# Python-for-HPC/ramba

Hardware: NVIDIA H100
Metric: fused-elementwise GB/s (fp64 sin/cos/mul/add chain) (higher is better)
Workload: dtype f64

## Files before the change

### ramba_b200/csrc/gen_handlers.py

```python
#!/usr/bin/env python

T = ["double", "float", "long long"]
BIN = ["RB200_OP_ADD", "RB200_OP_SUB", "RB200_OP_MUL"]
UN = ["RB200_OP_MOV", "RB200_OP_NEG", "RB200_OP_ABS", "RB200_OP_SQUARE", "RB200_OP_SQRT", "RB200_OP_SIN", "RB200_OP_COS",
      "RB200_OP_SINCOS", "RB200_OP_POWI"]
FLOAT_ONLY = {"RB200_OP_SQRT", "RB200_OP_SIN", "RB200_OP_COS", "RB200_OP_SINCOS", "RB200_OP_POWI"}

SETS = {
    1: dict(AK=["S_ACC", "S_REG", "S_PFV", "S_PFV32"], BK=["S_ACC", "S_REG", "S_SCAL", "S_PFV", "S_PFV32"]),
    2: dict(AK=["S_ACC", "S_REG", "S_VIEW", "S_VIEW32"], BK=["S_ACC", "S_REG", "S_SCAL", "S_VIEW", "S_VIEW32"]),
}


def carr(x):
    if isinstance(x, list):
        return "{" + ", ".join(carr(y) for y in x) + "}"
    return str(x)


tab = ["// GENERATED by gen_handlers.py — do not edit", "#pragma once", "namespace rb200 {"]
for sid, kinds in SETS.items():
    AK, BK = kinds["AK"], kinds["BK"]
    wide32 = {AK[3], BK[4]}
    cases = []
    hid = 0
    hbin = [[[[0] * len(BK) for _ in AK] for _ in T] for _ in BIN]
    hun = [[[0] * len(AK) for _ in T] for _ in UN]
    hred = [[0] * len(AK) for _ in range(2)]
    hcvt = [[[0] * len(AK) for _ in T] for _ in T]
    for ti, t in enumerate(T):
        for group in (lambda op: op not in ("RB200_OP_SIN", "RB200_OP_COS", "RB200_OP_SINCOS"), None,
                      lambda op: op in ("RB200_OP_SIN", "RB200_OP_COS", "RB200_OP_SINCOS")):
            if group is None:
                for oi, op in enumerate(BIN):
                    for ai, ak in enumerate(AK):
                        for bi, bk in enumerate(BK):
                            if (ak in wide32 or bk in wide32) and t != "double":
                                continue
                            hid += 1
                            hbin[oi][ti][ai][bi] = hid
                            cases.append((hid, f"h_bin<{op}, {t}, {ak}, {bk}, V>(cx, I); break;"))
                continue
            for oi, op in enumerate(UN):
                if not group(op):
                    continue
                if op in FLOAT_ONLY and t == "long long":
                    continue
                for ai, ak in enumerate(AK):
                    if ak in wide32 and t != "double":
                        continue
                    hid += 1
                    hun[oi][ti][ai] = hid
                    cases.append((hid, f"h_un<{op}, {t}, {ak}, V>(cx, I); break;"))
    for ti, t in enumerate(["double", "long long"]):
        for ai, ak in enumerate(AK):
            if ak in wide32 and t != "double":
                continue
            hid += 1
            hred[ti][ai] = hid
            cases.append((hid, f"h_red<{t}, {ak}, V, AX, NS>(cx, I, racc); break;"))
    for si, ts in enumerate(T):
        for di, td in enumerate(T):
            if si == di:
                continue
            for ai, ak in enumerate(AK[:3]):
                hid += 1
                hcvt[si][di][ai] = hid
                cases.append((hid, f"h_cvt<{ts}, {td}, {ak}, V>(cx, I); break;"))
    groups = {}
    for n, stmt in cases:
        groups.setdefault(n >> 4, []).append((n & 15, stmt))
    lines = ["// GENERATED by gen_handlers.py — do not edit", "switch (h >> 4) {"]
    for gi in sorted(groups):
        lines.append(f"  case {gi}:")
        lines.append("    switch (h & 15) {")
        for lo, stmt in groups[gi]:
            lines.append(f"      case {lo}: {stmt}")
        lines.append("      default: break;")
        lines.append("    }")
        lines.append("    break;")
    lines.append("  default: break;")
    lines.append("}")
    open(f"rb200_handlers_set{sid}.inc", "w").write("\n".join(lines) + "\n")
    tab += [f"// ---- set {sid}: a kinds {AK}, b kinds {BK}",
            f"constexpr int kNumHandlers{sid} = {hid};",
            f"static const short kHandlerBin{sid}[{len(BIN)}][{len(T)}][{len(AK)}][{len(BK)}] = {carr(hbin)};",
            f"static const short kHandlerUn{sid}[{len(UN)}][{len(T)}][{len(AK)}] = {carr(hun)};",
            f"static const short kHandlerRed{sid}[2][{len(AK)}] = {carr(hred)};",
            f"static const short kHandlerCvt{sid}[{len(T)}][{len(T)}][{len(AK)}] = {carr(hcvt)};"]
    print("set", sid, hid, "handlers")
tab += ["}  // namespace rb200", ""]
open("rb200_handler_tables.h", "w").write("\n".join(tab))
```

### ramba_b200/csrc/rb200_api.cu

```cuda
#include <cuda_runtime.h>
#include <math.h>
#include <stdio.h>
#include <stdlib.h>
#include <string.h>
#include <atomic>
#include <string>

#include "rb200_launch.h"
#include "rb200_handlers.h"
#include "rb200_group.h"
#include "rb200_index.h"
#include "rb200_rng.h"
#include "rb200_stream.h"
#include "rb200_tile.h"

namespace rb200 {
__global__ void fill_u64_kernel(u64* p, long long n, u64 bits) {
  for (long long i = (long long)blockIdx.x * blockDim.x + threadIdx.x; i < n; i += (long long)gridDim.x * blockDim.x) p[i] = bits;
}

template <class T> __global__ void reduce_partials_kernel(T* out, const T* part, long long n, long long k, long long stride_k, int op) {
  for (long long j = (long long)blockIdx.x * blockDim.x + threadIdx.x; j < n; j += (long long)gridDim.x * blockDim.x) {
    T v = part[j];
    for (long long q = 1; q < k; ++q) v = red_combine<T>(op, v, part[q * stride_k + j]);
    out[j] = v;
  }
}

}

using namespace rb200;

static thread_local std::string g_last_error;
static std::atomic<long long> g_launches{0};

static int fail(const std::string& msg) {
  g_last_error = msg;
  return 1;
}
static int fail_cuda(const char* what, cudaError_t e) {
  g_last_error = std::string(what) + ": " + cudaGetErrorString(e);
  return 2;
}

static int dtype_size(int dt) {
  switch (dt) {
    case RB200_F64:
    case RB200_I64: return 8;
    case RB200_F32:
    case RB200_I32:
    case RB200_U32: return 4;
    case RB200_I16:
    case RB200_U16: return 2;
    case RB200_BOOL:
    case RB200_U8:
    case RB200_I8: return 1;
    default: return 0;
  }
}

static std::atomic<int> g_sm_count{0};
static int sm_count() {
  const int cached = g_sm_count.load();
  if (cached > 0) return cached;
  int dev = 0;
  if (cudaGetDevice(&dev) != cudaSuccess) return -1;
  int n = 0;
  if (cudaDeviceGetAttribute(&n, cudaDevAttrMultiProcessorCount, dev) != cudaSuccess) return -1;
  g_sm_count.store(n);
  return n;
}

constexpr int kRedScratchPartials = 4096;

static int static_kind(const KParams& P, int set, int kind, int* idx, int ctype) {
  switch (kind) {
    case RB200_K_ACC: return S_ACC;
    case RB200_K_REG: return S_REG;
    case RB200_K_SCAL: return S_SCAL;
    case RB200_K_VIEW: {
      const KView& v = P.views[*idx];
      const int own = ctype == RB200_T_F64 ? RB200_F64 : ctype == RB200_T_F32 ? RB200_F32 : RB200_I64;
      if (set == 2) {
        if (v.dtype == own) return S_VIEW;
        if (ctype == RB200_T_F64 && v.dtype == RB200_F32) return S_VIEW32;
        return -1;
      }
      if (v.pf_slot < 0) return -1;
      if (v.dtype == own) {
        *idx = v.pf_slot;
        return S_PFV;
      }
      if (ctype == RB200_T_F64 && v.dtype == RB200_F32) {
        *idx = v.pf_slot;
        return S_PFV32;
      }
      return -1;
    }
    default: return -1;
  }
}

static unsigned long long host_red_identity_bits(int op, int ctype) {
  if (ctype == RB200_T_F64) {
    double d = (op == RB200_RED_ADD) ? 0.0 : (op == RB200_RED_MUL) ? 1.0 : (op == RB200_RED_MIN) ? INFINITY : -INFINITY;
    unsigned long long b;
    memcpy(&b, &d, 8);
    return b;
  }
  long long i = (op == RB200_RED_ADD) ? 0ll : (op == RB200_RED_MUL) ? 1ll : (op == RB200_RED_MIN) ? 0x7fffffffffffffffll : (long long)0x8000000000000000ull;
  return (unsigned long long)i;
}

static void assign_handlers(KParams& P, const rb200_fused_op* op, int set) {
  for (int i = 0; i < P.n_insns; ++i) {
    rb200_insn I = P.insns[i];
    int h = H_GENERIC;
    int ai = I.a_idx, bi = I.b_idx;
    const int ak = static_kind(P, set, I.a_kind, &ai, I.op == RB200_OP_CVT ? (int)(I.imm & 0xff) : (int)I.ctype);
    if (I.op == RB200_OP_ADD || I.op == RB200_OP_SUB || I.op == RB200_OP_MUL) {
      const int bk = static_kind(P, set, I.b_kind, &bi, I.ctype);
      h = handler_bin(set, I.op, I.ctype, ak, bk);
    } else if (I.op == RB200_OP_RED) {
      h = handler_red(set, I.ctype, ak);
    } else if (I.op == RB200_OP_CVT) {
      if ((I.imm >> 8) == 0) h = handler_cvt(set, (int)(I.imm & 0xff), I.ctype, ak);
    } else if (I.op == RB200_OP_POWI) {
      if (I.b_kind == RB200_K_SCAL && (long long)op->scalars[I.b_idx] == 2) h = handler_un(set, I.op, I.ctype, ak);
    } else if ((I.c_kind == RB200_K_NONE || I.op == RB200_OP_SINCOS) && I.b_kind == RB200_K_NONE) {
      h = handler_un(set, I.op, I.ctype, ak);
    }
    if (h != H_GENERIC) {
      I.a_idx = (uint8_t)ai;
      if (I.op != RB200_OP_RED) I.b_idx = (uint8_t)bi;
      P.insns[i] = I;
    }
    P.handler[i] = (unsigned short)h;
  }
}

struct KillSwitches {
  bool no_tile, no_stream, no_mapred, no_terms, no_tma, no_row_mode, no_rng;
};
static const KillSwitches& kill_switches() {
  static const KillSwitches k = {getenv("RB200_NO_TILE_KERNEL") != nullptr,   getenv("RB200_NO_STREAM_KERNEL") != nullptr,
                                 getenv("RB200_NO_MAPRED_KERNEL") != nullptr, getenv("RB200_NO_TERMS_KERNEL") != nullptr,
                                 getenv("RB200_NO_TMA") != nullptr,           getenv("RB200_NO_ROW_MODE") != nullptr,
                                 getenv("RB200_NO_RNG") != nullptr};
  return k;
}

static int validate(const rb200_fused_op* op, bool* empty) {
  if (!op) return fail("null fused op");
  if (op->abi_version != RB200_ABI_VERSION) return fail("ABI version mismatch between caller and libramba_b200");
  if (op->ndim < 1 || op->ndim > RB200_MAX_DIMS) return fail("ndim out of range");
  if (op->n_views < 0 || op->n_views > RB200_MAX_VIEWS) return fail("too many views");
  if (op->n_scalars < 0 || op->n_scalars > RB200_MAX_SCALARS) return fail("too many scalars");
  if (op->n_insns < 0 || op->n_insns > RB200_MAX_INSNS) return fail("too many instructions");
  if (op->n_regs < 0 || op->n_regs > RB200_MAX_REGS) return fail("too many spill registers");
  if (op->n_reds < 0 || op->n_reds > RB200_MAX_REDS) return fail("too many reductions");
  long long total = 1;
  for (int d = 0; d < op->ndim; ++d) {
    if (op->itershape[d] < 0) return fail("negative itershape");
    if (op->ndim > 1 && op->itershape[d] >= (1ll << 31)) return fail("N-d iteration dims must be < 2^31");
    total *= op->itershape[d];
  }
  *empty = total == 0 || op->n_insns == 0;
  if (*empty) return 0;

  for (int i = 0; i < op->n_insns; ++i) {
    const rb200_insn& I = op->insns[i];
    if (I.op >= RB200_NUM_OPS) return fail("bad opcode");
    if (I.ctype > RB200_T_I64) return fail("bad compute class");
    const uint8_t kinds[3] = {I.a_kind, I.b_kind, I.c_kind};
    const uint8_t idxs[3] = {I.a_idx, I.b_idx, I.c_idx};
    for (int q = 0; q < 3; ++q) {
      if (I.op == RB200_OP_RED && q == 1) continue;
      if (I.op == RB200_OP_SINCOS && q == 2) {
        if (kinds[q] == RB200_K_VIEW && idxs[q] >= op->n_views) return fail("view index out of range");
        continue;
      }
      switch (kinds[q]) {
        case RB200_K_NONE:
        case RB200_K_ACC: break;
        case RB200_K_REG: if (idxs[q] >= op->n_regs) return fail("register index out of range"); break;
        case RB200_K_VIEW: if (idxs[q] >= op->n_views) return fail("view index out of range"); break;
        case RB200_K_SCAL: if (idxs[q] >= op->n_scalars) return fail("scalar index out of range"); break;
        case RB200_K_IOTA: if (idxs[q] >= op->ndim) return fail("iota dim out of range"); break;
        default: return fail("bad operand kind");
      }
    }
    if (I.st_reg != RB200_NOSTORE && I.st_reg >= op->n_regs) return fail("st_reg out of range");
    if (I.st_view != RB200_NOSTORE && I.st_view >= op->n_views) return fail("st_view out of range");
    if (I.mask_reg != RB200_NOSTORE && I.mask_reg >= op->n_regs) return fail("mask_reg out of range");
    if (I.op == RB200_OP_SINCOS && I.st2 >= op->n_regs) return fail("sincos st2 out of range");
    if (I.op == RB200_OP_RED && I.b_idx >= op->n_reds) return fail("reduction slot out of range");
    if (I.op == RB200_OP_PHILOX) {
      if (I.imm > RB200_PHILOX_INTEGER) return fail("philox: bad output form");
      const int cls = I.imm == RB200_PHILOX_UNIFORM32 ? RB200_T_F32 : I.imm == RB200_PHILOX_INTEGER ? RB200_T_I64 : RB200_T_F64;
      if (I.ctype != cls) return fail("philox: compute class does not match the output form");
      if (I.a_kind != RB200_K_IOTA && I.a_kind != RB200_K_ACC && I.a_kind != RB200_K_REG) return fail("philox: the index must be an index, the accumulator or a register");
      if (I.b_kind != RB200_K_SCAL) return fail("philox: the key must be a scalar");
      if (I.imm == RB200_PHILOX_INTEGER) {
        if (I.c_kind != RB200_K_SCAL) return fail("philox: the integer form needs a scalar bound");
        if ((long long)op->scalars[I.c_idx] <= 0) return fail("philox: the bound must be positive");
      }
    }
  }
  for (int i = 0; i < op->n_views; ++i) {
    if (dtype_size(op->views[i].dtype) == 0) return fail("bad view dtype");
    if (!op->views[i].base) return fail("null view base pointer");
  }
  if (op->n_axis_red_dims != 0) {
    if (op->n_axis_red_dims >= op->ndim) return fail("axis reduction needs at least one kept dim");
    if (op->n_reds < 1) return fail("axis reduction without reduction slots");
    if (!op->red_scratch) return fail("axis reduction needs a partial buffer");
  } else if (op->n_reds > 0) {
    if (!op->red_scratch) return fail("global reduction needs red_scratch");
    for (int s = 0; s < op->n_reds; ++s) {
      if (!op->reds[s].out) return fail("null reduction output");
      if (dtype_size(op->reds[s].out_dtype) == 0) return fail("bad reduction output dtype");
      if (op->reds[s].ctype != RB200_T_F64 && op->reds[s].ctype != RB200_T_I64) return fail("reduction class must be F64 or I64");
    }
  }
  return 0;
}

enum PlanForm { FORM_NONE, FORM_TILE, FORM_STREAM, FORM_AXIS_AS_1D, FORM_AXIS_REDUCE, FORM_ELEMENTWISE, FORM_RNG };

struct Plan {
  PlanForm form;
  TilePlan tile;
  StreamPlan stream;
  RngPlan rng;
  KParams k;
  long long blocks;
  size_t smem;
  int n_split, n_written;
  long long kept;
  u64* partials;
  u64 identity;
};

static bool plan_axis_as_1d(const rb200_fused_op* op, int sms, const bool* view_read, size_t reg_bytes, Plan& pl) {
  const KParams& P = pl.k;
  const long long TILE1 = (long long)kThreads * kV1;
  const long long red_len = P.red_len, kept = P.total;
  bool ok = (op->ndim == 2 && P.red_ndim == 1 && op->n_reds == 1 && kept % TILE1 == 0 && kept / TILE1 <= (long long)sms * 2 && red_len >= 2);
  for (int i = 0; i < op->n_insns && ok; ++i) {
    const rb200_insn& I = op->insns[i];
    if (I.a_kind == RB200_K_IOTA || I.b_kind == RB200_K_IOTA || I.c_kind == RB200_K_IOTA) ok = false;
    if (I.st_view != RB200_NOSTORE) ok = false;
    if (I.op == RB200_OP_SINCOS && I.c_kind == RB200_K_VIEW) ok = false;
  }
  for (int i = 0; i < op->n_views && ok; ++i) {
    const rb200_view& v = op->views[i];
    if (!view_read[i]) continue;
    if (v.stride[1] != 1 || !(v.stride[0] == kept || v.stride[0] == 0)) ok = false;
  }
  if (!ok) return false;
  KParams Q = P;
  const int V1 = kV1;
  Q.ndim = 1;
  Q.total = red_len * kept;
  Q.n_tiles = Q.total / TILE1;
  Q.shape[0] = Q.total;
  Q.gstart[0] = 0;
  Q.wide = 1;
  const int n_chunks = (int)(kept / TILE1);
  long long cap1 = (long long)sms * 2;
  int n_split_eff = (int)(cap1 / n_chunks);
  if (n_split_eff > P.n_split) n_split_eff = P.n_split;
  if ((long long)n_split_eff > red_len) n_split_eff = (int)red_len;
  if (n_split_eff < 1) n_split_eff = 1;
  Q.n_split_chunks = n_chunks;
  Q.n_split = n_split_eff;
  Q.red_len = kept;
  Q.n_pf = 0;
  for (int i = 0; i < op->n_views; ++i) {
    KView& k = Q.views[i];
    const rb200_view& v = op->views[i];
    k.stride[0] = 1;
    k.pf_slot = -1;
    if (!view_read[i]) continue;
    const int dt = v.dtype;
    const bool wide_ok = (dt == RB200_F64 || dt == RB200_F32 || dt == RB200_I64 || dt == RB200_I32);
    if (v.stride[0] == 0) {
      k.pf_slot = -2;
    } else if (wide_ok && Q.n_pf < kMaxPf && reg_bytes + (size_t)(Q.n_pf + 1) * 2 * V1 * kThreads * 8 <= 108 * 1024) {
      k.pf_slot = Q.n_pf;
      Q.pf_view[Q.n_pf] = i;
      Q.n_pf++;
    }
  }
  for (int i = 0; i < op->n_views && Q.n_hoist < kMaxPf; ++i) {
    if (Q.views[i].pf_slot != -2 || Q.n_regs >= RB200_MAX_REGS) continue;
    int cls = -1;
    bool same = true;
    for (int q = 0; q < Q.n_insns; ++q) {
      const rb200_insn& I = Q.insns[q];
      const int use_cls = (I.op == RB200_OP_CVT) ? (int)(I.imm & 0xff) : (int)I.ctype;
      const bool uses = (I.a_kind == RB200_K_VIEW && I.a_idx == i) || (I.b_kind == RB200_K_VIEW && I.b_idx == i && I.op != RB200_OP_RED) ||
                        (I.c_kind == RB200_K_VIEW && I.c_idx == i && I.op != RB200_OP_SINCOS);
      if (!uses) continue;
      if (I.op == RB200_OP_POWI && I.b_kind == RB200_K_VIEW && I.b_idx == i) same = false;
      if (cls < 0) cls = use_cls;
      else if (cls != use_cls) same = false;
    }
    if (cls < 0 || !same) continue;
    const int r = Q.n_regs++;
    Q.hoist_view[Q.n_hoist] = i;
    Q.hoist_reg[Q.n_hoist] = r;
    Q.hoist_cls[Q.n_hoist] = cls;
    Q.n_hoist++;
    for (int q = 0; q < Q.n_insns; ++q) {
      rb200_insn& I = Q.insns[q];
      if (I.a_kind == RB200_K_VIEW && I.a_idx == i) { I.a_kind = RB200_K_REG; I.a_idx = (uint8_t)r; }
      if (I.b_kind == RB200_K_VIEW && I.b_idx == i && I.op != RB200_OP_RED) { I.b_kind = RB200_K_REG; I.b_idx = (uint8_t)r; }
      if (I.c_kind == RB200_K_VIEW && I.c_idx == i && I.op != RB200_OP_SINCOS) { I.c_kind = RB200_K_REG; I.c_idx = (uint8_t)r; }
    }
  }
  const size_t reg_bytes1 = (size_t)(Q.n_regs + 1) * V1 * kThreads * 8;
  Q.bulk = Q.n_pf > 0 ? 1 : 0;
  for (int j = 0; j < Q.n_pf; ++j)
    if ((((uintptr_t)op->views[Q.pf_view[j]].base) & 15u) != 0) Q.bulk = 0;
  Q.n_stages = 2;
  const size_t pf_bytes1 = (size_t)Q.n_pf * Q.n_stages * V1 * kThreads * 8;
  if (reg_bytes1 + pf_bytes1 > 200 * 1024) return false;
  assign_handlers(Q, op, 1);
  pl.k = Q;
  pl.form = FORM_AXIS_AS_1D;
  pl.blocks = (long long)n_split_eff * n_chunks;
  pl.smem = reg_bytes1 + pf_bytes1;
  pl.n_written = n_split_eff;
  return true;
}

static void make_plan(const rb200_fused_op* op, int sms, Plan& pl) {
  const KillSwitches& ks = kill_switches();
  pl.form = FORM_NONE;
  pl.n_split = pl.n_written = 0;
  if (!ks.no_rng && plan_rng(op, sms, pl.rng)) {
    pl.form = FORM_RNG;
    return;
  }
  if (!ks.no_tile && plan_stencil_tile(op, sms, !ks.no_terms, !ks.no_tma, pl.tile)) {
    pl.form = FORM_TILE;
    return;
  }
  if (op->ndim == 1 && op->n_axis_red_dims == 0 && !ks.no_stream &&
      plan_stream(op, sms, kRedScratchPartials, 0, !ks.no_terms, !ks.no_mapred, pl.stream)) {
    pl.form = FORM_STREAM;
    return;
  }

  const int V = (op->ndim == 1 && op->n_axis_red_dims == 0) ? kV1 : kV;
  const long long TILE = (long long)kThreads * V;
  KParams& P = pl.k;
  memset(&P, 0, sizeof(P));
  P.ndim = op->ndim;
  P.n_insns = op->n_insns;
  P.n_views = op->n_views;
  P.n_regs = op->n_regs;
  P.n_reds = op->n_reds;
  long long total = 1;
  for (int d = 0; d < op->ndim; ++d) {
    P.shape[d] = op->itershape[d];
    P.gstart[d] = op->global_start[d];
    total *= op->itershape[d];
  }
  bool view_read[RB200_MAX_VIEWS] = {false}, view_masked[RB200_MAX_VIEWS] = {false};
  for (int i = 0; i < op->n_insns; ++i) {
    const rb200_insn& I = op->insns[i];
    const uint8_t kinds[3] = {I.a_kind, I.b_kind, I.c_kind};
    const uint8_t idxs[3] = {I.a_idx, I.b_idx, I.c_idx};
    for (int q = 0; q < 3; ++q)
      if (kinds[q] == RB200_K_VIEW && !(I.op == RB200_OP_RED && q == 1) && !(I.op == RB200_OP_SINCOS && q == 2)) view_read[idxs[q]] = true;
    if (I.st_view != RB200_NOSTORE && I.mask_reg != RB200_NOSTORE) view_masked[I.st_view] = true;
    P.insns[i] = I;
  }
  for (int i = 0; i < op->n_scalars; ++i) P.scalars[i] = op->scalars[i];
  for (int i = 0; i < op->n_views; ++i) {
    const rb200_view& v = op->views[i];
    KView& k = P.views[i];
    k.base = (char*)v.base;
    k.dtype = v.dtype;
    k.pf_slot = -1;
    for (int d = 0; d < op->ndim; ++d) k.stride[d] = v.stride[d];
  }
  const size_t reg_bytes = (size_t)(op->n_regs + 1) * V * kThreads * 8;

  if (op->n_axis_red_dims != 0) {
    const int nred = op->n_axis_red_dims;
    P.red_ndim = nred;
    long long red_len = 1, kept = 1;
    for (int d = 0; d < nred; ++d) red_len *= P.shape[d];
    for (int d = nred; d < op->ndim; ++d) kept *= P.shape[d];
    int n_split = op->axis_nsplit;
    if (n_split < 1) n_split = 1;
    if ((long long)n_split > red_len) n_split = (int)red_len;
    P.red_len = red_len;
    P.n_split = n_split;
    P.red_split = (red_len + n_split - 1) / n_split;
    P.total = kept;
    P.n_tiles = ((kept + TILE - 1) / TILE) * n_split;
    P.red_partials = (u64*)op->red_scratch;
    for (int s = 0; s < op->n_reds; ++s) {
      P.reds[s].op = op->reds[s].op;
      P.reds[s].ctype = op->reds[s].ctype;
    }
    pl.n_split = n_split;
    pl.kept = kept;
    pl.partials = (u64*)op->red_scratch;
    pl.identity = host_red_identity_bits(op->reds[0].op, op->reds[0].ctype);
    if (!ks.no_stream && plan_stream(op, sms, kRedScratchPartials, n_split, !ks.no_terms, !ks.no_mapred, pl.stream)) {
      pl.form = FORM_STREAM;
      pl.n_written = pl.stream.eff;
      return;
    }
    if (plan_axis_as_1d(op, sms, view_read, reg_bytes, pl)) return;
    long long blocks = P.n_tiles;
    long long cap = (long long)sms * 4;
    if (blocks > cap) blocks = cap;
    pl.form = FORM_AXIS_REDUCE;
    pl.blocks = blocks;
    pl.smem = reg_bytes;
    pl.n_written = n_split;
    return;
  }

  P.total = total;
  P.n_tiles = (total + TILE - 1) / TILE;
  P.row_chunks = 0;
  if (op->ndim > 1) {
    const long long inner = op->itershape[op->ndim - 1];
    const long long chunks = (inner + TILE - 1) / TILE;
    if (!ks.no_row_mode && inner * 5 >= chunks * TILE * 4 && chunks < (1ll << 30)) {
      P.row_chunks = (int)chunks;
      P.n_tiles = (total / inner) * chunks;
    }
  }
  P.wide = (total >= (1ll << 31)) ? 1 : 0;
  size_t pf_bytes = 0;
  if (op->ndim == 1) {
    for (int i = 0; i < op->n_views && P.n_pf < kMaxPf; ++i) {
      const int dt = op->views[i].dtype;
      const bool wide_ok = (dt == RB200_F64 || dt == RB200_F32 || dt == RB200_I64 || dt == RB200_I32);
      if (view_read[i] && !view_masked[i] && wide_ok && reg_bytes + (size_t)(P.n_pf + 1) * 2 * V * kThreads * 8 <= 108 * 1024) {
        P.views[i].pf_slot = P.n_pf;
        P.pf_view[P.n_pf] = i;
        P.n_pf++;
      }
    }
    P.n_stages = 2;
    pf_bytes = (size_t)P.n_pf * P.n_stages * V * kThreads * 8;
    P.bulk = P.n_pf > 0 ? 1 : 0;
    for (int j = 0; j < P.n_pf; ++j) {
      const rb200_view& v = op->views[P.pf_view[j]];
      if (v.stride[0] != 1 || (((uintptr_t)v.base) & 15u) != 0) P.bulk = 0;
    }
  }
  size_t ocls_bytes = 0;
  if (op->ndim > 1) {
    for (int i = 0; i < op->n_views; ++i) {
      int c = -1;
      for (int q = 0; q < P.n_ocls && c < 0; ++q) {
        bool same = true;
        for (int d = 0; d < op->ndim; ++d)
          if (op->views[P.ocls_view[q]].stride[d] != op->views[i].stride[d]) same = false;
        if (same) c = q;
      }
      if (c < 0 && P.n_ocls < kMaxOcls) {
        c = P.n_ocls;
        P.ocls_view[P.n_ocls++] = i;
      }
      P.views[i].pf_slot = c;
    }
    ocls_bytes = (size_t)P.n_ocls * V * kThreads * 8;
  }
  const size_t smem = reg_bytes + pf_bytes + ocls_bytes;
  assign_handlers(P, op, op->ndim == 1 ? 1 : 2);
  if (op->n_reds > 0) {
    P.red_counter = (unsigned int*)op->red_scratch;
    P.red_partials = (u64*)((char*)op->red_scratch + 256);
    for (int s = 0; s < op->n_reds; ++s) {
      P.reds[s].op = op->reds[s].op;
      P.reds[s].ctype = op->reds[s].ctype;
      P.reds[s].out = op->reds[s].out;
      P.reds[s].out_dtype = op->reds[s].out_dtype;
    }
  }
  int per_sm = (V == 4 && op->ndim == 1) ? 3 : 2;
  if (smem > 0) {
    int by_smem = (int)((220 * 1024) / (smem + 1024));
    if (by_smem < 1) by_smem = 1;
    if (per_sm > by_smem) per_sm = by_smem;
  }
  long long blocks = P.n_tiles;
  long long cap = (long long)sms * per_sm;
  if (op->n_reds > 0 && cap > kRedScratchPartials) cap = kRedScratchPartials;
  if (blocks > cap) blocks = cap;
  pl.form = FORM_ELEMENTWISE;
  pl.blocks = blocks;
  pl.smem = smem;
}

static std::string launch_failure(const Plan& pl) {
  const KParams& P = pl.k;
  char buf[256];
  switch (pl.form) {
    case FORM_TILE: {
      const TilePlan& T = pl.tile;
      snprintf(buf, sizeof(buf), "stencil_tile_kernel launch (blocks=%lld smem=%zu group=%d tma=%d)", T.blocks, T.smem, T.P.has_group, T.P.use_tma);
    } break;
    case FORM_STREAM: {
      const StreamPlan& T = pl.stream;
      snprintf(buf, sizeof(buf), "stream kernel%s launch (blocks=%lld smem=%zu staged=%d depth=%d terms=%d)", T.P.mode == 1 ? " (columns)" : "", T.blocks,
               T.smem, T.P.n_staged, T.P.depth, T.P.n_terms);
    } break;
    case FORM_RNG: snprintf(buf, sizeof(buf), "rng_fill_kernel launch (blocks=%lld)", pl.rng.blocks); break;
    case FORM_AXIS_AS_1D: return "vm_elementwise_kernel (axis-as-1-D) launch";
    case FORM_AXIS_REDUCE: return "vm_axis_reduce_kernel launch";
    default:
      snprintf(buf, sizeof(buf), "vm_elementwise_kernel launch (ndim=%d blocks=%lld smem=%zu n_regs=%d n_pf=%d n_insns=%d)", P.ndim, pl.blocks, pl.smem,
               P.n_regs, P.n_pf, P.n_insns);
  }
  return buf;
}

static int launch(Plan& pl, cudaStream_t stream) {
  const KParams& P = pl.k;
  const unsigned blocks = (unsigned)pl.blocks;
  cudaError_t e = cudaSuccess;
  switch (pl.form) {
    case FORM_NONE: return 0;
    case FORM_TILE: e = launch_stencil_tile(pl.tile, stream); break;
    case FORM_STREAM: e = launch_stream(pl.stream, stream); break;
    case FORM_RNG: e = launch_rng(pl.rng, stream); break;
    case FORM_AXIS_AS_1D: e = launch_vm_elementwise_ax1d(P, blocks, pl.smem, stream); break;
    case FORM_AXIS_REDUCE: e = launch_vm_axis_reduce(P, blocks, pl.smem, stream); break;
    case FORM_ELEMENTWISE:
      switch (P.ndim) {
        case 1: e = launch_vm_elementwise_nd1(P, blocks, pl.smem, stream); break;
        case 2: e = launch_vm_elementwise_nd2(P, blocks, pl.smem, stream); break;
        case 3: e = launch_vm_elementwise_nd3(P, blocks, pl.smem, stream); break;
        default: e = launch_vm_elementwise_nd5(P, blocks, pl.smem, stream); break;
      }
      break;
  }
  if (e != cudaSuccess) return fail_cuda(launch_failure(pl).c_str(), e);
  g_launches.fetch_add(1);
  if (pl.n_written < pl.n_split) {
    const long long n_fill = (long long)(pl.n_split - pl.n_written) * pl.kept;
    fill_u64_kernel<<<(unsigned)((n_fill + 255) / 256 > 1184 ? 1184 : (n_fill + 255) / 256), 256, 0, stream>>>(pl.partials + (long long)pl.n_written * pl.kept,
                                                                                                               n_fill, pl.identity);
    e = cudaGetLastError();
    if (e != cudaSuccess) return fail_cuda("fill_u64_kernel launch", e);
    g_launches.fetch_add(1);
  }
  return 0;
}

static std::string describe(const rb200_fused_op* op, const Plan& pl) {
  if (pl.form == FORM_TILE) return describe_stencil_tile(pl.tile);
  if (pl.form == FORM_STREAM) return describe_stream(pl.stream);
  if (pl.form == FORM_RNG) return describe_rng(pl.rng);
  if (pl.form == FORM_NONE) return "kernel=none";
  const char* form = pl.form == FORM_ELEMENTWISE ? "elementwise" : pl.form == FORM_AXIS_AS_1D ? "axis_as_1d" : "axis_reduce";
  const char* tiling = pl.form != FORM_ELEMENTWISE || op->ndim == 1 ? "" : pl.k.row_chunks > 0 ? " tiling=row" : " tiling=flat";
  char buf[200];
  snprintf(buf, sizeof(buf), "kernel=general_interpreter form=%s ndim=%d insns=%d views=%d%s ctas=%lld smem=%zu", form, op->ndim, op->n_insns, op->n_views,
           tiling, pl.blocks, pl.smem);
  return buf;
}

static int check_index_view(const rb200_index_view* v, const char* who) {
  const std::string w(who);
  if (!v) return fail(w + ": null view");
  if (v->elem_bytes != 1 && v->elem_bytes != 2 && v->elem_bytes != 4 && v->elem_bytes != 8) return fail(w + ": elem_bytes must be 1, 2, 4 or 8");
  if (v->ndim < 1 || v->ndim > RB200_MAX_DIMS) return fail(w + ": ndim out of range");
  long long size = 1, lo = 0, hi = 0;
  for (int d = 0; d < v->ndim; ++d) {
    if (v->shape[d] < 0) return fail(w + ": negative shape");
    size *= v->shape[d];
    const long long reach = (v->shape[d] > 0 ? v->shape[d] - 1 : 0) * v->stride[d];
    if (reach < 0) lo += reach;
    else hi += reach;
  }
  if (size == 0) return 0;
  if (!v->base) return fail(w + ": null view base pointer");
  if (v->alloc_lo && v->alloc_hi) {
    const char* b = (const char*)v->base;
    if (b + lo * v->elem_bytes < (const char*)v->alloc_lo || b + (hi + 1) * v->elem_bytes > (const char*)v->alloc_hi)
      return fail(w + ": view outside its allocation");
  }
  return 0;
}

static int check_route_table(const rb200_route_table* t, RouteParams* R) {
  if (!t) return fail("route: null table");
  if (t->ndim < 1 || t->ndim > RB200_MAX_DIMS) return fail("route: ndim out of range");
  if (t->n_ranks < 1 || t->n_ranks > RB200_MAX_ROUTE_RANKS) return fail("route: too many ranks (or none)");
  if (!t->cuts || !t->cell_owner || !t->cell_offset || !t->cell_stride) return fail("route: null table array");
  R->ndim = t->ndim;
  R->n_ranks = t->n_ranks;
  R->size = 1;
  long long n_cells = 1;
  int n_cuts = 0;
  for (int d = 0; d < t->ndim; ++d) {
    if (t->shape[d] < 0) return fail("route: negative shape");
    if (t->n_cells[d] < 1) return fail("route: not a grid (no cells along a dim)");
    R->shape[d] = t->shape[d];
    R->size *= t->shape[d];
    n_cells *= t->n_cells[d];
    R->n_cells[d] = t->n_cells[d];
    R->cut_start[d] = n_cuts;
    const int first = t->cut_start[d], m = t->n_cells[d] + 1;
    if (first < 0 || n_cuts + m > RB200_MAX_ROUTE_CUTS) return fail("route: too many cut points");
    if (n_cells > RB200_MAX_ROUTE_CELLS) return fail("route: too many cells");
    for (int j = 0; j < m; ++j) R->cuts[n_cuts + j] = t->cuts[first + j];
    if (R->cuts[n_cuts] != 0 || R->cuts[n_cuts + m - 1] != t->shape[d]) return fail("route: not a grid (cuts must run from 0 to the extent)");
    for (int j = 1; j < m; ++j)
      if (R->cuts[n_cuts + j] <= R->cuts[n_cuts + j - 1] && t->shape[d] > 0) return fail("route: not a grid (cuts must ascend)");
    n_cuts += m;
  }
  for (long long c = 0; c < n_cells; ++c) {
    if (t->cell_owner[c] < 0 || t->cell_owner[c] >= t->n_ranks) return fail("route: cell owner out of range");
    R->owner[c] = t->cell_owner[c];
    R->offset[c] = t->cell_offset[c];
    for (int d = 0; d < t->ndim; ++d) R->stride[c * t->ndim + d] = t->cell_stride[c * t->ndim + d];
  }
  return 0;
}

static int check_group_args(const rb200_index_view* src, int axis, int n_groups, GroupPlan* P) {
  if (const int rc = check_index_view(src, "group_reduce")) return rc;
  if (axis < 0 || axis >= src->ndim) return fail("group_reduce: axis out of range");
  if (n_groups < 1) return fail("group_reduce: n_groups must be >= 1");
  make_group_plan(*src, axis, n_groups, P);
  if (P->ctas >= (1ll << 31)) return fail("group_reduce: too many outputs for one launch");
  return 0;
}

static thread_local std::string g_group_plan_text;

extern "C" {

const char* rb200_last_error(void) { return g_last_error.c_str(); }
int rb200_abi_version(void) { return RB200_ABI_VERSION; }
int64_t rb200_launch_count(void) { return (int64_t)g_launches.load(); }
void rb200_reset_launch_count(void) { g_launches.store(0); }
int rb200_device_sm_count(void) { return sm_count(); }
int64_t rb200_red_scratch_bytes(void) { return (int64_t)(256 + 8 * RB200_MAX_REDS * kRedScratchPartials); }

int rb200_run_deferred_ops(const rb200_fused_op* op, void* stream_v) {
  bool empty = false;
  if (const int rc = validate(op, &empty)) return rc;
  if (empty) return 0;
  const int sms = sm_count();
  if (sms <= 0) return fail("no usable CUDA device (libramba_b200 has no CPU path)");
  Plan pl;
  make_plan(op, sms, pl);
  return launch(pl, (cudaStream_t)stream_v);
}

int rb200_describe_plan(const rb200_fused_op* op, char* out, int64_t cap) {
  if (!out || cap < 2) return fail("describe_plan: null argument");
  bool empty = false;
  if (const int rc = validate(op, &empty)) return rc;
  Plan pl;
  pl.form = FORM_NONE;
  if (!empty) make_plan(op, 132, pl);
  snprintf(out, (size_t)cap, "%s", describe(op, pl).c_str());
  return 0;
}

int64_t rb200_cumulative_scratch_bytes(int64_t n_outer, int64_t len, int64_t n_inner) {
  if (n_outer < 0 || len < 0 || n_inner < 1) return 256;
  return (int64_t)scan_scratch_bytes(n_outer, len, n_inner);
}

int rb200_cumulative(const void* src, void* dst, int32_t dtype, int64_t n_outer, int64_t len, int64_t n_inner, int32_t redop, const void* carry_in,
                     void* totals_out, void* scratch, void* stream_v) {
  if (n_outer < 0 || len < 0 || n_inner < 1) return fail("cumulative: bad extents");
  if (redop < RB200_RED_ADD || redop > RB200_RED_MAX) return fail("cumulative: bad operation");
  if (dtype != RB200_F64 && dtype != RB200_F32 && dtype != RB200_I64 && dtype != RB200_I32) return fail("cumulative: dtype must be float64/float32/int64/int32");
  if (n_outer == 0 || len == 0) return 0;
  if (!src || !dst || !scratch) return fail("null pointer");
  const int sms = sm_count();
  if (sms <= 0) return fail("no usable CUDA device (libramba_b200 has no CPU path)");
  bool supported = true;
  const cudaError_t e = launch_scan(src, dst, dtype, n_outer, len, n_inner, redop, carry_in, totals_out, scratch, sms, (cudaStream_t)stream_v, &supported);
  if (!supported) return fail("cumulative: unsupported dtype");
  if (e != cudaSuccess) return fail_cuda("scan kernel launch", e);
  g_launches.fetch_add(1);
  return 0;
}

int rb200_gather(const rb200_index_view* view, const int64_t* lin, int64_t n, void* out, uint64_t* bad, void* stream_v) {
  if (const int rc = check_index_view(view, "gather")) return rc;
  if (n < 0) return fail("gather: negative n");
  if (n == 0) return 0;
  if (!lin || !out || !bad) return fail("gather: null pointer");
  const int sms = sm_count();
  if (sms <= 0) return fail("no usable CUDA device (libramba_b200 has no CPU path)");
  const cudaError_t e = launch_gather(collapse_index_view(*view), (const long long*)lin, n, out, (unsigned long long*)bad, sms, (cudaStream_t)stream_v);
  if (e != cudaSuccess) return fail_cuda("gather kernel launch", e);
  g_launches.fetch_add(1);
  return 0;
}

int rb200_scatter(const rb200_index_view* view, const int64_t* lin, int64_t n, const void* values, uint64_t* bad, void* stream_v) {
  if (const int rc = check_index_view(view, "scatter")) return rc;
  if (n < 0) return fail("scatter: negative n");
  if (n == 0) return 0;
  if (!lin || !values || !bad) return fail("scatter: null pointer");
  const int sms = sm_count();
  if (sms <= 0) return fail("no usable CUDA device (libramba_b200 has no CPU path)");
  const cudaError_t e =
      launch_scatter(collapse_index_view(*view), (const long long*)lin, n, values, (unsigned long long*)bad, sms, (cudaStream_t)stream_v);
  if (e != cudaSuccess) return fail_cuda("scatter kernel launch", e);
  g_launches.fetch_add(1);
  return 0;
}

int64_t rb200_route_scratch_bytes(int64_t n, int32_t n_ranks) {
  if (n < 0 || n_ranks < 1) return 256;
  return (int64_t)route_scratch_bytes(n, n_ranks);
}

int rb200_route(const rb200_route_table* table, const int64_t* lin, int64_t n, int64_t* offsets, int64_t* slots, int64_t* counts, uint64_t* bad,
                void* scratch, void* stream_v) {
  RouteParams R;
  if (const int rc = check_route_table(table, &R)) return rc;
  if (n < 0) return fail("route: negative n");
  if (!counts || !scratch) return fail("route: null pointer");
  if (n > 0 && (!lin || !offsets || !slots || !bad)) return fail("route: null pointer");
  const int sms = sm_count();
  if (sms <= 0) return fail("no usable CUDA device (libramba_b200 has no CPU path)");
  const cudaError_t e = launch_route(R, (const long long*)lin, n, (long long*)offsets, (long long*)slots, (long long*)counts,
                                     (unsigned long long*)bad, scratch, sms, (cudaStream_t)stream_v);
  if (e != cudaSuccess) return fail_cuda("route kernel launch", e);
  g_launches.fetch_add(1);
  return 0;
}

int64_t rb200_group_reduce_scratch_bytes(const rb200_index_view* src, int32_t axis, int32_t n_groups) {
  GroupPlan P;
  if (check_group_args(src, axis, n_groups, &P)) return -1;
  return (int64_t)P.scratch_bytes;
}

const char* rb200_describe_group_plan(const rb200_index_view* src, int32_t axis, int32_t n_groups) {
  GroupPlan P;
  if (check_group_args(src, axis, n_groups, &P)) return nullptr;
  char buf[240];
  snprintf(buf, sizeof(buf), "kernel=group form=%s chunk=%lld chunks=%d cta_chunks=%d ctas_per_row=%d kept=%lld groups=%d ctas=%lld scratch=%lld",
           group_form_name(P.form), P.C, P.S, P.ncl, P.K, P.nkept, P.G, P.ctas, P.scratch_bytes);
  g_group_plan_text = buf;
  return g_group_plan_text.c_str();
}

int rb200_group_reduce(const rb200_index_view* src, int32_t src_dtype, int32_t axis, const rb200_group_table* groups, int32_t op, const void* center,
                       void* out, void* scratch, void* stream_v) {
  if (op < 0 || op >= RB200_GROUP_NUM_OPS) return fail("group_reduce: bad op");
  if (src_dtype != RB200_F64 && src_dtype != RB200_F32 && src_dtype != RB200_I64 && src_dtype != RB200_I32)
    return fail("group_reduce: source dtype must be float64, float32, int64 or int32");
  if (src && dtype_size(src_dtype) != src->elem_bytes) return fail("group_reduce: elem_bytes does not match the source dtype");
  if (!groups) return fail("group_reduce: null group table");
  GroupPlan P;
  if (const int rc = check_group_args(src, axis, groups->n_groups, &P)) return rc;
  if (groups->len != src->shape[axis]) return fail("group_reduce: table len differs from the extent of the grouped axis");
  if (!groups->offsets || (groups->len > 0 && !groups->members)) return fail("group_reduce: null table array");
  if (op == RB200_GROUP_SQDEV && !center) return fail("group_reduce: SQDEV needs center");
  if (!out) return fail("group_reduce: null out");
  if (P.scratch_bytes && !scratch) return fail("group_reduce: null scratch (this plan splits the axis)");
  if (P.nkept == 0) return 0;
  const int sms = sm_count();
  if (sms <= 0) return fail("no usable CUDA device (libramba_b200 has no CPU path)");
  const cudaError_t e = launch_group(P, src_dtype, op, (const long long*)groups->offsets, (const long long*)groups->members, (const double*)center, out,
                                     scratch, (cudaStream_t)stream_v);
  if (e != cudaSuccess) return fail_cuda("group kernel launch", e);
  g_launches.fetch_add(1);
  return 0;
}

int rb200_reduce_partials(void* out, const void* partials, int64_t n, int64_t k, int64_t stride_k, int32_t dtype,
                          int32_t redop, void* stream_v) {
  if (!out || !partials) return fail("null pointer");
  if (n <= 0 || k <= 0) return 0;
  const int sms = sm_count();
  if (sms <= 0) return fail("no usable CUDA device (libramba_b200 has no CPU path)");
  cudaStream_t stream = (cudaStream_t)stream_v;
  long long blocks = (n + 255) / 256;
  if (blocks > sms * 8) blocks = sms * 8;
  if (dtype == RB200_F64)
    reduce_partials_kernel<double><<<(unsigned)blocks, 256, 0, stream>>>((double*)out, (const double*)partials, n, k, stride_k, redop);
  else if (dtype == RB200_I64)
    reduce_partials_kernel<long long><<<(unsigned)blocks, 256, 0, stream>>>((long long*)out, (const long long*)partials, n, k, stride_k, redop);
  else
    return fail("reduce_partials: dtype must be F64 or I64 (accumulator classes)");
  cudaError_t e = cudaGetLastError();
  if (e != cudaSuccess) return fail_cuda("reduce_partials_kernel launch", e);
  g_launches.fetch_add(1);
  return 0;
}

}
```

### ramba_b200/csrc/rb200_elementwise.cuh

```cuda
#pragma once
#include "rb200_interp.cuh"
#include "rb200_launch.h"

namespace rb200 {

template <int V, int ND, bool AX1D = false>
#ifndef RB200_MIN_BLOCKS
#define RB200_MIN_BLOCKS 2
#endif
__global__ void __launch_bounds__(kThreads, (ND == 1 && V <= 4) ? 3 : RB200_MIN_BLOCKS) vm_elementwise_kernel(const __grid_constant__ KParams P) {
  extern __shared__ __align__(128) unsigned char smem[];
  __shared__ __align__(8) u64 mbar_store[4];
  constexpr int TILE = kThreads * V;
  constexpr unsigned SLOT = (unsigned)(TILE * 8);
  Ctx<V, ND> cx(P);
  const unsigned smem_s = (unsigned)__cvta_generic_to_shared(smem);
  cx.tid = threadIdx.x;
  const int n_pf = (ND == 1) ? P.n_pf : 0;
  const unsigned pf_base = smem_s;
  const unsigned pf_stage_bytes = (unsigned)n_pf * SLOT;
  const bool bulk = (ND == 1) && n_pf > 0 && P.bulk;
  constexpr unsigned S = 2u;
  cx.regfile_s = smem_s + (n_pf > 0 ? S : 0u) * pf_stage_bytes + threadIdx.x * 8u;
  cx.ocls_s = cx.regfile_s + (unsigned)((P.n_regs + 1) * V * kThreads * 8);
  cx.pf_s = pf_base;
  const unsigned mbar0 = (unsigned)__cvta_generic_to_shared(&mbar_store[0]);
  if (bulk) {
    if (threadIdx.x == 0) {
      for (unsigned s = 0; s < S; ++s) mbar_init(mbar0 + s * 8u, 1);
      asm volatile("fence.mbarrier_init.release.cluster;" ::: "memory");
    }
    __syncthreads();
  }

  constexpr int NS = 1;
  __shared__ u64 racc_extra[RB200_MAX_REDS - 1][kThreads];
  u64 racc[NS][AX1D ? V : 1];
#pragma unroll
  for (int k = 0; k < (AX1D ? V : 1); ++k) racc[0][k] = red_identity_bits(0 < P.n_reds ? P.reds[0].op : 0, 0 < P.n_reds ? P.reds[0].ctype : 0);
  cx.racc_s = (unsigned)__cvta_generic_to_shared(&racc_extra[0][threadIdx.x]);
  for (int s = 1; s < P.n_reds; ++s) racc_extra[s - 1][threadIdx.x] = red_identity_bits(P.reds[s].op, P.reds[s].ctype);
  if constexpr (AX1D) {
    cx.pe0 = (long long)(blockIdx.x % (unsigned)P.n_split_chunks) * TILE + threadIdx.x;
    cx.e0 = cx.pe0;
    cx.valid = (1u << V) - 1u;
#pragma unroll 1
    for (int h = 0; h < P.n_hoist; ++h) {
      const KView& vw = P.views[P.hoist_view[h]];
      long long off[V];
      cx.offsets(vw, off);
      u64 bits[V];
      if (P.hoist_cls[h] == RB200_T_F64) {
        double t[V];
        load_view<double, V>(vw.base, vw.dtype, off, cx.valid, t);
#pragma unroll
        for (int k = 0; k < V; ++k) bits[k] = CT<double>::bits(t[k]);
      } else if (P.hoist_cls[h] == RB200_T_F32) {
        float t[V];
        load_view<float, V>(vw.base, vw.dtype, off, cx.valid, t);
#pragma unroll
        for (int k = 0; k < V; ++k) bits[k] = CT<float>::bits(t[k]);
      } else {
        long long t[V];
        load_view<long long, V>(vw.base, vw.dtype, off, cx.valid, t);
#pragma unroll
        for (int k = 0; k < V; ++k) bits[k] = CT<long long>::bits(t[k]);
      }
      sts_vec64<V>(cx.reg_base(P.hoist_reg[h]), bits);
    }
  } else {
    cx.pe0 = 0;
  }

  auto issue_bulk = [&](long long t, unsigned st) {
    const unsigned mb = mbar0 + st * 8u;
    unsigned bytes = 0;
#pragma unroll 1
    for (int j = 0; j < n_pf; ++j) {
      const int dt = P.views[P.pf_view[j]].dtype;
      bytes += (unsigned)TILE * ((dt == RB200_F64 || dt == RB200_I64) ? 8u : 4u);
    }
    mbar_expect_tx(mb, bytes);
#pragma unroll 1
    for (int j = 0; j < n_pf; ++j) {
      const KView& vw = P.views[P.pf_view[j]];
      const unsigned es = (vw.dtype == RB200_F64 || vw.dtype == RB200_I64) ? 8u : 4u;
      bulk_g2s(pf_base + st * pf_stage_bytes + (unsigned)j * SLOT, vw.base + t * (long long)TILE * es, (unsigned)TILE * es, mb);
    }
  };
  auto issue_ldgsts = [&](long long t, unsigned st) {
    const long long e0 = t * TILE + threadIdx.x;
    const long long left = P.total - e0;
#pragma unroll 1
    for (int j = 0; j < n_pf; ++j) {
      const KView& vw = P.views[P.pf_view[j]];
      const int es = (vw.dtype == RB200_F64 || vw.dtype == RB200_I64) ? 8 : 4;
      const long long sb = vw.stride[0] * es;
      const long long step = sb * kThreads;
      const char* src = vw.base + e0 * sb;
      unsigned dst = pf_base + st * pf_stage_bytes + (unsigned)j * SLOT + threadIdx.x * (unsigned)es;
#pragma unroll
      for (int k = 0; k < V; ++k) {
        const bool ok = (long long)k * kThreads < left;
        if (es == 8) cp_async8(dst, ok ? src : vw.base, ok);
        else cp_async4(dst, ok ? src : vw.base, ok);
        src += step;
        dst += (unsigned)(kThreads * es);
      }
    }
  };
  auto tile_is_bulk = [&](long long t) { return bulk && (t + 1) * TILE <= P.total; };

  constexpr unsigned lgS = 1u;
  if (n_pf > 0 && (long long)blockIdx.x < P.n_tiles) {
    if (bulk) {
      if (threadIdx.x == 0) {
        long long t = blockIdx.x;
        for (unsigned s = 0; s < S && t < P.n_tiles; ++s, t += gridDim.x)
          if (tile_is_bulk(t)) issue_bulk(t, s);
      }
    } else {
      issue_ldgsts(blockIdx.x, 0);
      cp_async_commit();
    }
  }
#pragma unroll 1
  for (unsigned it = 0;; ++it) {
    unsigned grid = gridDim.x;
    asm volatile("" : "+r"(grid));
    const long long tile = (long long)blockIdx.x + (long long)it * grid;
    if (tile >= P.n_tiles) break;
    const unsigned stage = bulk ? (it & (S - 1u)) : (it & 1u);
    if (n_pf > 0) {
      if (bulk) {
        __syncthreads();
        if (it > 0 && threadIdx.x == 0) {
          const long long nxt = tile + (long long)(S - 1u) * grid;
          if (nxt < P.n_tiles && tile_is_bulk(nxt)) issue_bulk(nxt, (it - 1u) & (S - 1u));
        }
        if (tile_is_bulk(tile)) {
          mbar_wait(mbar0 + stage * 8u, (it >> lgS) & 1u);
        } else {
          issue_ldgsts(tile, stage);
          cp_async_commit();
          cp_async_wait<0>();
        }
      } else {
        const long long nxt = tile + grid;
        if (nxt < P.n_tiles) issue_ldgsts(nxt, stage ^ 1u);
        cp_async_commit();
        cp_async_wait<1>();
      }
      cx.pf_s = pf_base + stage * pf_stage_bytes;
    }
    const long long e0 = tile * TILE + threadIdx.x;
    unsigned valid = 0;
    if constexpr (ND == 1) {
      cx.e0 = e0;
      if ((tile + 1) * TILE <= P.total) {
        valid = (1u << V) - 1u;
      } else {
#pragma unroll
        for (int k = 0; k < V; ++k)
          if (e0 + (long long)k * kThreads < P.total) valid |= (1u << k);
      }
    } else if (P.row_chunks > 0) {
      long long row, ch;
      if (((tile | (long long)P.row_chunks) >> 31) == 0) row = (long long)((unsigned)tile / (unsigned)P.row_chunks);
      else row = tile / P.row_chunks;
      ch = tile - row * P.row_chunks;
      long long oidx[ND];
#pragma unroll
      for (int d = ND - 1; d >= 0; --d) {
        if (d >= P.ndim - 1) {
          oidx[d] = 0;
        } else if (d == 0) {
          oidx[d] = row;
        } else {
          const long long sd = P.shape[d];
          long long q;
          if (((row | sd) >> 31) == 0) q = (long long)((unsigned)row / (unsigned)sd);
          else q = row / sd;
          oidx[d] = row - q * sd;
          row = q;
        }
      }
      const long long inner = P.shape[P.ndim - 1];
      const long long j0 = ch * TILE + threadIdx.x;
#pragma unroll
      for (int k = 0; k < V; ++k) {
        const long long j = j0 + (long long)k * kThreads;
        const bool ok = j < inner;
        if (ok) valid |= (1u << k);
#pragma unroll
        for (int d = 0; d < ND; ++d) cx.idx[k][d] = (d == P.ndim - 1) ? (ok ? j : 0) : (ok ? oidx[d] : 0);
      }
    } else {
#pragma unroll
      for (int k = 0; k < V; ++k) {
        const long long e = e0 + (long long)k * kThreads;
        if (e < P.total) {
          valid |= (1u << k);
          decode_index<ND>(P, e, 0, cx.idx[k]);
        } else {
#pragma unroll
          for (int d = 0; d < ND; ++d) cx.idx[k][d] = 0;
        }
      }
    }
    cx.valid = valid;
    cx.fill_offset_classes();
    run_program<V, AX1D, NS>(cx, racc);
  }
  if (n_pf > 0 && !bulk) cp_async_wait<0>();

  if constexpr (AX1D) {
    const long long split = blockIdx.x / (unsigned)P.n_split_chunks;
    const long long col0 = cx.pe0;
#pragma unroll
    for (int k = 0; k < V; ++k) P.red_partials[split * P.red_len + col0 + (long long)k * kThreads] = racc[0][k];
    return;
  }
  if (P.n_reds > 0) {
    __shared__ u64 wpart[RB200_MAX_REDS][kThreads / 32];
    __shared__ bool is_last;
    const int lane = threadIdx.x & 31, warp = threadIdx.x >> 5;
    for (int s = 0; s < P.n_reds; ++s) {
      const int op = P.reds[s].op, ct = P.reds[s].ctype;
      u64 v = (s == 0) ? racc[0][0] : racc_extra[s > 0 ? s - 1 : 0][threadIdx.x];
#pragma unroll
      for (int o = 16; o > 0; o >>= 1) v = red_combine_bits(op, ct, v, __shfl_down_sync(0xffffffffu, v, o));
      if (lane == 0) wpart[s][warp] = v;
    }
    __syncthreads();
    if (threadIdx.x == 0) {
      for (int s = 0; s < P.n_reds; ++s) {
        const int op = P.reds[s].op, ct = P.reds[s].ctype;
        u64 v = wpart[s][0];
        for (int q = 1; q < kThreads / 32; ++q) v = red_combine_bits(op, ct, v, wpart[s][q]);
        P.red_partials[(long long)s * gridDim.x + blockIdx.x] = v;
      }
      __threadfence();
      unsigned prev = atomicAdd(P.red_counter, 1u);
      is_last = (prev == gridDim.x - 1);
    }
    __syncthreads();
    if (is_last) {
      __threadfence();
      for (int s = 0; s < P.n_reds; ++s) {
        const int op = P.reds[s].op, ct = P.reds[s].ctype;
        u64 v = red_identity_bits(op, ct);
        for (unsigned b = threadIdx.x; b < gridDim.x; b += kThreads) v = red_combine_bits(op, ct, v, __ldcg(&P.red_partials[(long long)s * gridDim.x + b]));
#pragma unroll
        for (int o = 16; o > 0; o >>= 1) v = red_combine_bits(op, ct, v, __shfl_down_sync(0xffffffffu, v, o));
        __syncthreads();
        if (lane == 0) wpart[s][warp] = v;
        __syncthreads();
        if (threadIdx.x == 0) {
          v = wpart[s][0];
          for (int q = 1; q < kThreads / 32; ++q) v = red_combine_bits(op, ct, v, wpart[s][q]);
          void* out = P.reds[s].out;
          const double vd = (ct == RB200_T_F64) ? CT<double>::get(v) : (double)(long long)v;
          const long long vi = (ct == RB200_T_F64) ? (long long)CT<double>::get(v) : (long long)v;
          switch (P.reds[s].out_dtype) {
            case RB200_F64: { double* o = (double*)out; *o = red_combine<double>(op, *o, vd); } break;
            case RB200_F32: { float* o = (float*)out; *o = (float)red_combine<double>(op, (double)*o, vd); } break;
            case RB200_I64: { long long* o = (long long*)out; *o = red_combine<long long>(op, *o, vi); } break;
            case RB200_I32: { int* o = (int*)out; *o = (int)red_combine<long long>(op, (long long)*o, vi); } break;
            case RB200_BOOL: { unsigned char* o = (unsigned char*)out; *o = red_combine<long long>(op, (long long)*o, vi) != 0 ? 1 : 0; } break;
            case RB200_U8: { unsigned char* o = (unsigned char*)out; *o = (unsigned char)red_combine<long long>(op, (long long)*o, vi); } break;
            case RB200_I8: { signed char* o = (signed char*)out; *o = (signed char)red_combine<long long>(op, (long long)*o, vi); } break;
            case RB200_I16: { short* o = (short*)out; *o = (short)red_combine<long long>(op, (long long)*o, vi); } break;
            case RB200_U16: { unsigned short* o = (unsigned short*)out; *o = (unsigned short)red_combine<long long>(op, (long long)*o, vi); } break;
            case RB200_U32: { unsigned int* o = (unsigned int*)out; *o = (unsigned int)red_combine<long long>(op, (long long)*o, vi); } break;
            default: break;
          }
        }
      }
      if (threadIdx.x == 0) *P.red_counter = 0u;
    }
  }
}

template <int V, int ND, bool AX1D = false> cudaError_t launch_vm_elementwise_nd(const KParams& P, unsigned blocks, size_t smem, cudaStream_t stream) {
  if (smem + 2048 > 48 * 1024) {
    cudaError_t e = cudaFuncSetAttribute(vm_elementwise_kernel<V, ND, AX1D>, cudaFuncAttributeMaxDynamicSharedMemorySize, (int)smem);
    if (e != cudaSuccess) return e;
  }
  vm_elementwise_kernel<V, ND, AX1D><<<blocks, kThreads, smem, stream>>>(P);
  return cudaGetLastError();
}

}
```

### ramba_b200/csrc/rb200_handler_tables.h

```cpp
#pragma once
namespace rb200 {
constexpr int kNumHandlers1 = 232;
static const short kHandlerBin1[3][3][4][5] = {{{{25, 26, 27, 28, 29}, {30, 31, 32, 33, 34}, {35, 36, 37, 38, 39}, {40, 41, 42, 43, 44}}, {{115, 116, 117, 118, 0}, {119, 120, 121, 122, 0}, {123, 124, 125, 126, 0}, {0, 0, 0, 0, 0}}, {{172, 173, 174, 175, 0}, {176, 177, 178, 179, 0}, {180, 181, 182, 183, 0}, {0, 0, 0, 0, 0}}}, {{{45, 46, 47, 48, 49}, {50, 51, 52, 53, 54}, {55, 56, 57, 58, 59}, {60, 61, 62, 63, 64}}, {{127, 128, 129, 130, 0}, {131, 132, 133, 134, 0}, {135, 136, 137, 138, 0}, {0, 0, 0, 0, 0}}, {{184, 185, 186, 187, 0}, {188, 189, 190, 191, 0}, {192, 193, 194, 195, 0}, {0, 0, 0, 0, 0}}}, {{{65, 66, 67, 68, 69}, {70, 71, 72, 73, 74}, {75, 76, 77, 78, 79}, {80, 81, 82, 83, 84}}, {{139, 140, 141, 142, 0}, {143, 144, 145, 146, 0}, {147, 148, 149, 150, 0}, {0, 0, 0, 0, 0}}, {{196, 197, 198, 199, 0}, {200, 201, 202, 203, 0}, {204, 205, 206, 207, 0}, {0, 0, 0, 0, 0}}}};
static const short kHandlerUn1[9][3][4] = {{{1, 2, 3, 4}, {97, 98, 99, 0}, {160, 161, 162, 0}}, {{5, 6, 7, 8}, {100, 101, 102, 0}, {163, 164, 165, 0}}, {{9, 10, 11, 12}, {103, 104, 105, 0}, {166, 167, 168, 0}}, {{13, 14, 15, 16}, {106, 107, 108, 0}, {169, 170, 171, 0}}, {{17, 18, 19, 20}, {109, 110, 111, 0}, {0, 0, 0, 0}}, {{85, 86, 87, 88}, {151, 152, 153, 0}, {0, 0, 0, 0}}, {{89, 90, 91, 92}, {154, 155, 156, 0}, {0, 0, 0, 0}}, {{93, 94, 95, 96}, {157, 158, 159, 0}, {0, 0, 0, 0}}, {{21, 22, 23, 24}, {112, 113, 114, 0}, {0, 0, 0, 0}}};
static const short kHandlerRed1[2][4] = {{208, 209, 210, 211}, {212, 213, 214, 0}};
static const short kHandlerCvt1[3][3][4] = {{{0, 0, 0, 0}, {215, 216, 217, 0}, {218, 219, 220, 0}}, {{221, 222, 223, 0}, {0, 0, 0, 0}, {224, 225, 226, 0}}, {{227, 228, 229, 0}, {230, 231, 232, 0}, {0, 0, 0, 0}}};
constexpr int kNumHandlers2 = 232;
static const short kHandlerBin2[3][3][4][5] = {{{{25, 26, 27, 28, 29}, {30, 31, 32, 33, 34}, {35, 36, 37, 38, 39}, {40, 41, 42, 43, 44}}, {{115, 116, 117, 118, 0}, {119, 120, 121, 122, 0}, {123, 124, 125, 126, 0}, {0, 0, 0, 0, 0}}, {{172, 173, 174, 175, 0}, {176, 177, 178, 179, 0}, {180, 181, 182, 183, 0}, {0, 0, 0, 0, 0}}}, {{{45, 46, 47, 48, 49}, {50, 51, 52, 53, 54}, {55, 56, 57, 58, 59}, {60, 61, 62, 63, 64}}, {{127, 128, 129, 130, 0}, {131, 132, 133, 134, 0}, {135, 136, 137, 138, 0}, {0, 0, 0, 0, 0}}, {{184, 185, 186, 187, 0}, {188, 189, 190, 191, 0}, {192, 193, 194, 195, 0}, {0, 0, 0, 0, 0}}}, {{{65, 66, 67, 68, 69}, {70, 71, 72, 73, 74}, {75, 76, 77, 78, 79}, {80, 81, 82, 83, 84}}, {{139, 140, 141, 142, 0}, {143, 144, 145, 146, 0}, {147, 148, 149, 150, 0}, {0, 0, 0, 0, 0}}, {{196, 197, 198, 199, 0}, {200, 201, 202, 203, 0}, {204, 205, 206, 207, 0}, {0, 0, 0, 0, 0}}}};
static const short kHandlerUn2[9][3][4] = {{{1, 2, 3, 4}, {97, 98, 99, 0}, {160, 161, 162, 0}}, {{5, 6, 7, 8}, {100, 101, 102, 0}, {163, 164, 165, 0}}, {{9, 10, 11, 12}, {103, 104, 105, 0}, {166, 167, 168, 0}}, {{13, 14, 15, 16}, {106, 107, 108, 0}, {169, 170, 171, 0}}, {{17, 18, 19, 20}, {109, 110, 111, 0}, {0, 0, 0, 0}}, {{85, 86, 87, 88}, {151, 152, 153, 0}, {0, 0, 0, 0}}, {{89, 90, 91, 92}, {154, 155, 156, 0}, {0, 0, 0, 0}}, {{93, 94, 95, 96}, {157, 158, 159, 0}, {0, 0, 0, 0}}, {{21, 22, 23, 24}, {112, 113, 114, 0}, {0, 0, 0, 0}}};
static const short kHandlerRed2[2][4] = {{208, 209, 210, 211}, {212, 213, 214, 0}};
static const short kHandlerCvt2[3][3][4] = {{{0, 0, 0, 0}, {215, 216, 217, 0}, {218, 219, 220, 0}}, {{221, 222, 223, 0}, {0, 0, 0, 0}, {224, 225, 226, 0}}, {{227, 228, 229, 0}, {230, 231, 232, 0}, {0, 0, 0, 0}}};
}
```

### ramba_b200/csrc/rb200_interp.cuh

```cuda
#pragma once
#include <cuda_runtime.h>
#include <math.h>
#include <type_traits>

#include "rb200_vm.cuh"
#include "rb200_handlers.h"
#include "rb200_philox.h"

namespace rb200 {

struct UInsn {
  uint2 lo, hi;
  __device__ __forceinline__ UInsn(const rb200_insn* p) {
    lo = *reinterpret_cast<const uint2*>(p);
    hi = *(reinterpret_cast<const uint2*>(p) + 1);
  }
  __device__ __forceinline__ unsigned op() const { return lo.x & 0xffu; }
  __device__ __forceinline__ unsigned ctype() const { return (lo.x >> 8) & 0xffu; }
  __device__ __forceinline__ unsigned a_kind() const { return (lo.x >> 16) & 0xffu; }
  __device__ __forceinline__ unsigned a_idx() const { return lo.x >> 24; }
  __device__ __forceinline__ unsigned b_kind() const { return lo.y & 0xffu; }
  __device__ __forceinline__ unsigned b_idx() const { return (lo.y >> 8) & 0xffu; }
  __device__ __forceinline__ unsigned c_kind() const { return (lo.y >> 16) & 0xffu; }
  __device__ __forceinline__ unsigned c_idx() const { return lo.y >> 24; }
  __device__ __forceinline__ unsigned st_reg() const { return hi.x & 0xffu; }
  __device__ __forceinline__ unsigned st_view() const { return (hi.x >> 8) & 0xffu; }
  __device__ __forceinline__ unsigned st2() const { return (hi.x >> 16) & 0xffu; }
  __device__ __forceinline__ unsigned mask_reg() const { return hi.x >> 24; }
  __device__ __forceinline__ unsigned imm() const { return hi.y; }
};

template <class T, int V, int K = 0> __device__ __forceinline__ void lds_vec64(unsigned base, T (&out)[V]) {
  if constexpr (K < V) {
    out[K] = CT<T>::get(lds64o<K * kThreads * 8>(base));
    lds_vec64<T, V, K + 1>(base, out);
  }
}
template <class T, int V, int K = 0> __device__ __forceinline__ void lds_vec32(unsigned base, T (&out)[V]) {
  if constexpr (K < V) {
    out[K] = CT<T>::get((u64)lds32o<K * kThreads * 4>(base));
    lds_vec32<T, V, K + 1>(base, out);
  }
}
template <int V, int K = 0> __device__ __forceinline__ void lds_vec32_as_f64(unsigned base, double (&out)[V]) {
  if constexpr (K < V) {
    out[K] = (double)__uint_as_float(lds32o<K * kThreads * 4>(base));
    lds_vec32_as_f64<V, K + 1>(base, out);
  }
}
template <int V, int K = 0> __device__ __forceinline__ void sts_vec64(unsigned base, const u64 (&v)[V]) {
  if constexpr (K < V) {
    sts64o<K * kThreads * 8>(base, v[K]);
    sts_vec64<V, K + 1>(base, v);
  }
}

template <class R>
__device__ __noinline__ void store_line(char* base, int dtype, long long off0, long long step, unsigned mask, u64 b0, u64 b1, u64 b2, u64 b3) {
  constexpr int V = 4;
  long long off[V] = {off0, off0 + step, off0 + 2 * step, off0 + 3 * step};
  R r[V] = {CT<R>::get(b0), CT<R>::get(b1), CT<R>::get(b2), CT<R>::get(b3)};
  constexpr int own = std::is_same<R, double>::value ? RB200_F64 : std::is_same<R, float>::value ? RB200_F32 : RB200_I64;
  if (dtype == own) {
    store_direct<R, R, V>(base, off, mask, r);
  } else if (dtype == RB200_BOOL) {
    long long b[V];
#pragma unroll
    for (int k = 0; k < V; ++k) b[k] = (r[k] != R(0)) ? 1 : 0;
    store_view<long long, V>(base, RB200_U8, off, mask, b);
  } else {
    store_view<R, V>(base, dtype, off, mask, r);
  }
}

template <class R> __device__ __forceinline__ void store_one(char* base, int dtype, long long off, R x) {
  switch (dtype) {
    case RB200_F64: reinterpret_cast<double*>(base)[off] = (double)x; break;
    case RB200_F32: reinterpret_cast<float*>(base)[off] = (float)x; break;
    case RB200_I64: reinterpret_cast<long long*>(base)[off] = (long long)x; break;
    case RB200_I32: reinterpret_cast<int*>(base)[off] = (int)x; break;
    default: store_narrow_one<R>(base, dtype, off, x);
  }
}

template <class R, int V>
__device__ __noinline__ void store_slow_1d(char* base, int dtype, long long stride, long long e0, unsigned valid, unsigned mask_addr,
                                           unsigned vals_addr) {
  const long long step = stride * kThreads;
  long long off = e0 * stride;
#pragma unroll 1
  for (int k = 0; k < V; ++k, off += step) {
    if (!((valid >> k) & 1u)) continue;
    if (mask_addr != 0xffffffffu && lds64(mask_addr + (unsigned)(k * kThreads * 8)) == 0ull) continue;
    store_one<R>(base, dtype, off, CT<R>::get(lds64(vals_addr + (unsigned)(k * kThreads * 8))));
  }
}

template <class R>
__device__ __noinline__ void store_slow_nd(char* base, int dtype, unsigned mask, long long o0, long long o1, long long o2, long long o3,
                                           unsigned vals_addr) {
  if (mask & 1u) store_one<R>(base, dtype, o0, CT<R>::get(lds64(vals_addr)));
  if (mask & 2u) store_one<R>(base, dtype, o1, CT<R>::get(lds64(vals_addr + (unsigned)(kThreads * 8))));
  if (mask & 4u) store_one<R>(base, dtype, o2, CT<R>::get(lds64(vals_addr + (unsigned)(2 * kThreads * 8))));
  if (mask & 8u) store_one<R>(base, dtype, o3, CT<R>::get(lds64(vals_addr + (unsigned)(3 * kThreads * 8))));
}

template <int V, int ND> struct Ctx {
  static constexpr int kND = ND;
  const KParams& P;
  unsigned regfile_s;
  unsigned racc_s;
  unsigned pf_s;
  unsigned ocls_s;
  unsigned tid;
  long long e0;
  long long pe0;
  long long idx[V][ND];
  unsigned valid;
  u64 acc[V];

  __device__ __forceinline__ Ctx(const KParams& p) : P(p) {}

  __device__ __forceinline__ void offsets(const KView& vw, long long (&off)[V]) const {
    if constexpr (ND == 1) {
      const long long s = vw.stride[0];
      const long long step = s * kThreads;
      long long o = (vw.pf_slot == -2 ? pe0 : e0) * s;
#pragma unroll
      for (int k = 0; k < V; ++k) {
        off[k] = o;
        o += step;
      }
    } else {
      const int c = vw.pf_slot;
      if (c >= 0) {
        lds_vec64<long long, V>(ocls_s + (unsigned)(c * V * kThreads * 8), off);
        return;
      }
      compute_offsets(vw, off);
    }
  }
  __device__ __forceinline__ void compute_offsets(const KView& vw, long long (&off)[V]) const {
    if constexpr (ND > 1) {
#pragma unroll
      for (int k = 0; k < V; ++k) {
        long long o = 0;
#pragma unroll
        for (int d = 0; d < ND; ++d) o += idx[k][d] * vw.stride[d];
        off[k] = o;
      }
    }
  }
  __device__ __forceinline__ void fill_offset_classes() {
    if constexpr (ND > 1) {
#pragma unroll 1
      for (int c = 0; c < P.n_ocls; ++c) {
        long long off[V];
        compute_offsets(P.views[P.ocls_view[c]], off);
        u64 b[V];
#pragma unroll
        for (int k = 0; k < V; ++k) b[k] = (u64)off[k];
        sts_vec64<V>(ocls_s + (unsigned)(c * V * kThreads * 8), b);
      }
    }
  }

  __device__ __forceinline__ unsigned reg_addr(int r, int k) const { return regfile_s + (unsigned)((r * V + k) * kThreads * 8); }
  __device__ __forceinline__ unsigned reg_base(int r) const { return regfile_s + (unsigned)(r * V * kThreads * 8); }

  template <class T> __device__ __forceinline__ void fetch(int kind, int i, T (&out)[V]) {
    switch (kind) {
      case RB200_K_ACC:
#pragma unroll
        for (int k = 0; k < V; ++k) out[k] = CT<T>::get(acc[k]);
        break;
      case RB200_K_REG:
#pragma unroll
        for (int k = 0; k < V; ++k) out[k] = CT<T>::get(lds64(reg_addr(i, k)));
        break;
      case RB200_K_VIEW: {
        const KView& vw = P.views[i];
        const int slot = vw.pf_slot;
        const int dt = vw.dtype;
        if (ND == 1 && slot >= 0) {
          const unsigned slot_s = pf_s + (unsigned)(slot * V * kThreads * 8);
#pragma unroll
          for (int k = 0; k < V; ++k) out[k] = staged_load<T>(slot_s, k * kThreads + (int)tid, dt);
        } else {
          long long off[V];
          offsets(vw, off);
          load_view<T, V>(vw.base, dt, off, valid, out);
        }
      } break;
      case RB200_K_SCAL: {
        T s = CT<T>::get(P.scalars[i]);
#pragma unroll
        for (int k = 0; k < V; ++k) out[k] = s;
      } break;
      case RB200_K_IOTA: {
        if constexpr (ND == 1) {
          long long base = e0 + P.gstart[0];
#pragma unroll
          for (int k = 0; k < V; ++k) out[k] = (T)(base + (long long)k * kThreads);
        } else {
          long long g = 0;
#pragma unroll
          for (int d = 0; d < ND; ++d)
            if (d == i) g = P.gstart[d];
#pragma unroll
          for (int k = 0; k < V; ++k) {
            long long x = 0;
#pragma unroll
            for (int d = 0; d < ND; ++d)
              if (d == i) x = idx[k][d];
            out[k] = (T)(x + g);
          }
        }
      } break;
      default:
#pragma unroll
        for (int k = 0; k < V; ++k) out[k] = T(0);
    }
  }

  template <class R> __device__ __forceinline__ void store_out(int view, const R (&r)[V], const u64 (&bits)[V], unsigned m) {
    const KView& vw = P.views[view];
    if constexpr (ND == 1 && V % 4 == 0) {
      const long long st = vw.stride[0];
      const long long step = st * kThreads;
      char* const base = vw.base;
      const int dt = vw.dtype;
      constexpr int own1 = std::is_same<R, double>::value ? RB200_F64 : std::is_same<R, float>::value ? RB200_F32 : RB200_I64;
      if (dt == own1 && st == 1 && m == ((1u << V) - 1u)) {
        R* p = reinterpret_cast<R*>(base) + e0;
#pragma unroll
        for (int k = 0; k < V; ++k) stg<R>(p + k * kThreads, r[k]);
        return;
      }
#pragma unroll
      for (int g = 0; g < V / 4; ++g)
        store_line<R>(base, dt, (e0 + (long long)g * 4 * kThreads) * st, step, (m >> (4 * g)) & 0xfu, bits[4 * g], bits[4 * g + 1],
                      bits[4 * g + 2], bits[4 * g + 3]);
    } else {
      long long off[V];
      offsets(vw, off);
      constexpr int own = std::is_same<R, double>::value ? RB200_F64 : std::is_same<R, float>::value ? RB200_F32 : RB200_I64;
      if (vw.dtype == own) {
        store_direct<R, R, V>(vw.base, off, m, r);
      } else if (vw.dtype == RB200_BOOL) {
        long long b[V];
#pragma unroll
        for (int k = 0; k < V; ++k) b[k] = (r[k] != R(0)) ? 1 : 0;
        store_view<long long, V>(vw.base, RB200_U8, off, m, b);
      } else {
        store_view<R, V>(vw.base, vw.dtype, off, m, r);
      }
    }
  }

  template <class R> __device__ __forceinline__ void store_res(int vi, int mreg, const R (&r)[V], const u64 (&b)[V]) {
    if constexpr (ND == 1 && (V == 4 || V == 8)) {
      const KView& vw = P.views[vi];
      constexpr int own1 = std::is_same<R, double>::value ? RB200_F64 : std::is_same<R, float>::value ? RB200_F32 : RB200_I64;
      const long long st = vw.stride[0];
      const bool plain = st == 1 && valid == ((1u << V) - 1u) && mreg == RB200_NOSTORE;
      if (plain && vw.dtype == own1) {
        R* p = reinterpret_cast<R*>(vw.base) + e0;
#pragma unroll
        for (int k = 0; k < V; ++k) stg<R>(p + k * kThreads, r[k]);
      } else if (std::is_same<R, double>::value && plain && vw.dtype == RB200_F32) {
        float* p = reinterpret_cast<float*>(vw.base) + e0;
#pragma unroll
        for (int k = 0; k < V; ++k) stg<float>(p + k * kThreads, (float)r[k]);
      } else {
        const unsigned maddr = mreg == RB200_NOSTORE ? 0xffffffffu : reg_base(mreg);
        sts_vec64<V>(reg_base(P.n_regs), b);
        store_slow_1d<R, V>(vw.base, vw.dtype, st, e0, valid, maddr, reg_base(P.n_regs));
      }
    } else if constexpr (ND > 1 && V == 4) {
      const KView& vw = P.views[vi];
      constexpr int own = std::is_same<R, double>::value ? RB200_F64 : std::is_same<R, float>::value ? RB200_F32 : RB200_I64;
      long long off[V];
      offsets(vw, off);
      const bool plain = valid == 0xfu && mreg == RB200_NOSTORE;
      if (plain && vw.dtype == own) {
        R* p = reinterpret_cast<R*>(vw.base);
#pragma unroll
        for (int k = 0; k < V; ++k) stg<R>(p + off[k], r[k]);
      } else if (std::is_same<R, double>::value && plain && vw.dtype == RB200_F32) {
        float* p = reinterpret_cast<float*>(vw.base);
#pragma unroll
        for (int k = 0; k < V; ++k) stg<float>(p + off[k], (float)r[k]);
      } else {
        unsigned m = valid;
        if (mreg != RB200_NOSTORE) {
#pragma unroll
          for (int k = 0; k < V; ++k)
            if (lds64(reg_addr(mreg, k)) == 0ull) m &= ~(1u << k);
        }
        sts_vec64<V>(reg_base(P.n_regs), b);
        store_slow_nd<R>(vw.base, vw.dtype, m, off[0], off[1], off[2], off[3], reg_base(P.n_regs));
      }
    } else {
      unsigned m = valid;
      if (mreg != RB200_NOSTORE) {
#pragma unroll
        for (int k = 0; k < V; ++k)
          if (lds64(reg_addr(mreg, k)) == 0ull) m &= ~(1u << k);
      }
      store_out<R>(vi, r, b, m);
    }
  }

  template <class R> __device__ __forceinline__ void finish(const UInsn& I, const R (&r)[V]) {
#pragma unroll
    for (int k = 0; k < V; ++k) acc[k] = CT<R>::bits(r[k]);
    if (I.st_reg() != RB200_NOSTORE) sts_vec64<V>(reg_base(I.st_reg()), acc);
    if (I.st_view() != RB200_NOSTORE) store_res<R>(I.st_view(), I.mask_reg(), r, acc);
  }
};

template <class F> __device__ __noinline__ F rare_float_binary(int op, F a, F b) {
  return op == RB200_OP_FLOORDIV ? py_ffloordiv<F>(a, b) : op == RB200_OP_MOD ? py_fmod<F>(a, b) : (F)pow(a, b);
}
template <class F> __device__ __noinline__ F rare_powi(F a, long long e) { return powi<F>(a, e); }
template <class F> __device__ __noinline__ F rare_float_unary(int op, F x) {
  return op == RB200_OP_TAN    ? tan(x)
         : op == RB200_OP_SINH ? sinh(x)
         : op == RB200_OP_COSH ? cosh(x)
         : op == RB200_OP_TANH ? tanh(x)
         : op == RB200_OP_ASIN ? asin(x)
         : op == RB200_OP_ACOS ? acos(x)
         : op == RB200_OP_ATAN ? atan(x)
         : op == RB200_OP_EXP  ? exp(x)
         : op == RB200_OP_LOG  ? log(x)
                               : cbrt(x);
}
static __device__ __noinline__ long long rare_int_binary(int op, long long a, long long b) {
  return op == RB200_OP_FLOORDIV ? py_floordiv(a, b) : op == RB200_OP_MOD ? py_mod(a, b) : ipowi(a, b);
}

template <class F, int V, class C> __device__ __forceinline__ void exec_float(C& cx, const UInsn& I) {
  F a[V], b[V], r[V];
  long long p[V];
  const int op = I.op();
  cx.template fetch<F>(I.a_kind(), I.a_idx(), a);
  if (I.b_kind() != RB200_K_NONE && op != RB200_OP_POWI) cx.template fetch<F>(I.b_kind(), I.b_idx(), b);
  switch (op) {
    case RB200_OP_ADD:
#pragma unroll
      for (int k = 0; k < V; ++k) {
        if constexpr (sizeof(F) == 8) r[k] = __dadd_rn(a[k], b[k]);
        else r[k] = __fadd_rn(a[k], b[k]);
      }
      cx.template finish<F>(I, r);
      return;
    case RB200_OP_SUB:
#pragma unroll
      for (int k = 0; k < V; ++k) {
        if constexpr (sizeof(F) == 8) r[k] = __dsub_rn(a[k], b[k]);
        else r[k] = __fsub_rn(a[k], b[k]);
      }
      cx.template finish<F>(I, r);
      return;
    case RB200_OP_MUL:
#pragma unroll
      for (int k = 0; k < V; ++k) {
        if constexpr (sizeof(F) == 8) r[k] = __dmul_rn(a[k], b[k]);
        else r[k] = __fmul_rn(a[k], b[k]);
      }
      cx.template finish<F>(I, r);
      return;
    case RB200_OP_DIV:
#pragma unroll
      for (int k = 0; k < V; ++k) {
        if constexpr (sizeof(F) == 8) r[k] = __ddiv_rn(a[k], b[k]);
        else r[k] = __fdiv_rn(a[k], b[k]);
      }
      cx.template finish<F>(I, r);
      return;
    case RB200_OP_MIN:
#pragma unroll
      for (int k = 0; k < V; ++k) r[k] = (b[k] < a[k]) ? b[k] : a[k];
      cx.template finish<F>(I, r);
      return;
    case RB200_OP_MAX:
#pragma unroll
      for (int k = 0; k < V; ++k) r[k] = (b[k] > a[k]) ? b[k] : a[k];
      cx.template finish<F>(I, r);
      return;
    case RB200_OP_FLOORDIV:
    case RB200_OP_MOD:
    case RB200_OP_POW:
#pragma unroll
      for (int k = 0; k < V; ++k) r[k] = rare_float_binary<F>(op, a[k], b[k]);
      cx.template finish<F>(I, r);
      return;
    case RB200_OP_POWI: {
      long long e[V];
      cx.template fetch<long long>(I.b_kind(), I.b_idx(), e);
      bool sq = true;
#pragma unroll
      for (int k = 0; k < V; ++k) sq = sq && (e[k] == 2);
      if (sq) {
#pragma unroll
        for (int k = 0; k < V; ++k) {
          if constexpr (sizeof(F) == 8) r[k] = __dmul_rn(a[k], a[k]);
          else r[k] = __fmul_rn(a[k], a[k]);
        }
      } else {
#pragma unroll
        for (int k = 0; k < V; ++k) r[k] = rare_powi<F>(a[k], e[k]);
      }
      cx.template finish<F>(I, r);
      return;
    }
    case RB200_OP_GT:
    case RB200_OP_LT:
    case RB200_OP_GE:
    case RB200_OP_LE:
    case RB200_OP_EQ:
    case RB200_OP_NE:
#pragma unroll
      for (int k = 0; k < V; ++k) {
        F x = a[k], y = b[k];
        bool t = op == RB200_OP_GT ? x > y : op == RB200_OP_LT ? x < y : op == RB200_OP_GE ? x >= y : op == RB200_OP_LE ? x <= y : op == RB200_OP_EQ ? x == y : x != y;
        p[k] = t ? 1 : 0;
      }
      cx.template finish<long long>(I, p);
      return;
    case RB200_OP_LAND:
    case RB200_OP_LOR:
    case RB200_OP_LXOR:
#pragma unroll
      for (int k = 0; k < V; ++k) {
        bool x = a[k] != F(0), y = b[k] != F(0);
        p[k] = (op == RB200_OP_LAND ? (x && y) : op == RB200_OP_LOR ? (x || y) : (x != y)) ? 1 : 0;
      }
      cx.template finish<long long>(I, p);
      return;
    case RB200_OP_ISFINITE:
    case RB200_OP_ISINF:
    case RB200_OP_ISNAN:
    case RB200_OP_ISNEGINF:
    case RB200_OP_ISPOSINF:
    case RB200_OP_LNOT:
#pragma unroll
      for (int k = 0; k < V; ++k) {
        F x = a[k];
        bool t = op == RB200_OP_ISFINITE ? isfinite(x)
                 : op == RB200_OP_ISINF  ? isinf(x)
                 : op == RB200_OP_ISNAN  ? isnan(x)
                 : op == RB200_OP_ISNEGINF ? (isinf(x) && x < F(0))
                 : op == RB200_OP_ISPOSINF ? (isinf(x) && x > F(0))
                                           : (x == F(0));
        p[k] = t ? 1 : 0;
      }
      cx.template finish<long long>(I, p);
      return;
    case RB200_OP_MOV:
#pragma unroll
      for (int k = 0; k < V; ++k) r[k] = a[k];
      cx.template finish<F>(I, r);
      return;
    case RB200_OP_ABS:
#pragma unroll
      for (int k = 0; k < V; ++k) r[k] = fabs(a[k]);
      cx.template finish<F>(I, r);
      return;
    case RB200_OP_NEG:
#pragma unroll
      for (int k = 0; k < V; ++k) r[k] = -a[k];
      cx.template finish<F>(I, r);
      return;
    case RB200_OP_SQUARE:
#pragma unroll
      for (int k = 0; k < V; ++k) {
        if constexpr (sizeof(F) == 8) r[k] = __dmul_rn(a[k], a[k]);
        else r[k] = __fmul_rn(a[k], a[k]);
      }
      cx.template finish<F>(I, r);
      return;
    case RB200_OP_SQRT:
#pragma unroll
      for (int k = 0; k < V; ++k) r[k] = sqrt(a[k]);
      cx.template finish<F>(I, r);
      return;
    case RB200_OP_SIN:
    case RB200_OP_COS:
    case RB200_OP_SINCOS: {
      F sn[V], cs[V];
      sincos_v<V>(a, sn, cs);
      const bool want_cos = (op == RB200_OP_COS) || (op == RB200_OP_SINCOS && I.imm());
#pragma unroll
      for (int k = 0; k < V; ++k) r[k] = want_cos ? cs[k] : sn[k];
      if (op == RB200_OP_SINCOS) {
        u64 park[V];
        F parkv[V];
#pragma unroll
        for (int k = 0; k < V; ++k) {
          parkv[k] = want_cos ? sn[k] : cs[k];
          park[k] = CT<F>::bits(parkv[k]);
        }
        sts_vec64<V>(cx.reg_base(I.st2()), park);
        if (I.c_kind() == RB200_K_VIEW) cx.template store_out<F>(I.c_idx(), parkv, park, cx.valid);
      }
      cx.template finish<F>(I, r);
      return;
    }
    case RB200_OP_TAN:
    case RB200_OP_SINH:
    case RB200_OP_COSH:
    case RB200_OP_TANH:
    case RB200_OP_ASIN:
    case RB200_OP_ACOS:
    case RB200_OP_ATAN:
    case RB200_OP_EXP:
    case RB200_OP_LOG:
    case RB200_OP_CBRT:
#pragma unroll
      for (int k = 0; k < V; ++k) r[k] = rare_float_unary<F>(op, a[k]);
      cx.template finish<F>(I, r);
      return;
    case RB200_OP_WHERE: {
      F c[V];
      cx.template fetch<F>(I.c_kind(), I.c_idx(), c);
#pragma unroll
      for (int k = 0; k < V; ++k) r[k] = (a[k] != F(0)) ? b[k] : c[k];
      cx.template finish<F>(I, r);
      return;
    }
    case RB200_OP_MULADD:
    case RB200_OP_MULSUB:
    case RB200_OP_MULRSUB: {
      F c[V];
      cx.template fetch<F>(I.c_kind(), I.c_idx(), c);
#pragma unroll
      for (int k = 0; k < V; ++k) {
        if constexpr (sizeof(F) == 8) {
          const double p = __dmul_rn(b[k], c[k]);
          r[k] = op == RB200_OP_MULADD ? __dadd_rn(a[k], p) : op == RB200_OP_MULSUB ? __dsub_rn(a[k], p) : __dsub_rn(p, a[k]);
        } else {
          const float p = __fmul_rn(b[k], c[k]);
          r[k] = op == RB200_OP_MULADD ? __fadd_rn(a[k], p) : op == RB200_OP_MULSUB ? __fsub_rn(a[k], p) : __fsub_rn(p, a[k]);
        }
      }
      cx.template finish<F>(I, r);
      return;
    }
    default: return;
  }
}

template <int V, class C> __device__ __forceinline__ void exec_int(C& cx, const UInsn& I) {
  long long a[V], b[V], r[V];
  cx.template fetch<long long>(I.a_kind(), I.a_idx(), a);
  if (I.b_kind() != RB200_K_NONE) cx.template fetch<long long>(I.b_kind(), I.b_idx(), b);
  const int op = I.op();
  switch (op) {
    case RB200_OP_MOV:
#pragma unroll
      for (int k = 0; k < V; ++k) r[k] = a[k];
      break;
    case RB200_OP_ADD:
#pragma unroll
      for (int k = 0; k < V; ++k) r[k] = a[k] + b[k];
      break;
    case RB200_OP_SUB:
#pragma unroll
      for (int k = 0; k < V; ++k) r[k] = a[k] - b[k];
      break;
    case RB200_OP_MUL:
#pragma unroll
      for (int k = 0; k < V; ++k) r[k] = a[k] * b[k];
      break;
    case RB200_OP_MIN:
    case RB200_OP_MAX:
    case RB200_OP_BAND:
    case RB200_OP_BOR:
    case RB200_OP_BXOR:
    case RB200_OP_SHL:
    case RB200_OP_SHR:
#pragma unroll
      for (int k = 0; k < V; ++k) {
        long long x = a[k], y = b[k];
        r[k] = op == RB200_OP_MIN ? ((y < x) ? y : x)
               : op == RB200_OP_MAX ? ((y > x) ? y : x)
               : op == RB200_OP_BAND ? (x & y)
               : op == RB200_OP_BOR  ? (x | y)
               : op == RB200_OP_BXOR ? (x ^ y)
               : op == RB200_OP_SHL  ? (long long)((u64)x << (y & 63))
                                     : (x >> (y & 63));
      }
      break;
    case RB200_OP_FLOORDIV:
    case RB200_OP_MOD:
    case RB200_OP_POWI:
    case RB200_OP_POW:
#pragma unroll
      for (int k = 0; k < V; ++k) r[k] = rare_int_binary(op == RB200_OP_POW ? RB200_OP_POWI : op, a[k], b[k]);
      break;
    case RB200_OP_GT:
    case RB200_OP_LT:
    case RB200_OP_GE:
    case RB200_OP_LE:
    case RB200_OP_EQ:
    case RB200_OP_NE:
    case RB200_OP_LAND:
    case RB200_OP_LOR:
    case RB200_OP_LXOR:
#pragma unroll
      for (int k = 0; k < V; ++k) {
        long long x = a[k], y = b[k];
        bool t = op == RB200_OP_GT   ? x > y
                 : op == RB200_OP_LT ? x < y
                 : op == RB200_OP_GE ? x >= y
                 : op == RB200_OP_LE ? x <= y
                 : op == RB200_OP_EQ ? x == y
                 : op == RB200_OP_NE ? x != y
                 : op == RB200_OP_LAND ? (x != 0 && y != 0)
                 : op == RB200_OP_LOR  ? (x != 0 || y != 0)
                                       : ((x != 0) != (y != 0));
        r[k] = t ? 1 : 0;
      }
      break;
    case RB200_OP_ABS:
#pragma unroll
      for (int k = 0; k < V; ++k) r[k] = a[k] < 0 ? -a[k] : a[k];
      break;
    case RB200_OP_NEG:
#pragma unroll
      for (int k = 0; k < V; ++k) r[k] = -a[k];
      break;
    case RB200_OP_SQUARE:
#pragma unroll
      for (int k = 0; k < V; ++k) r[k] = a[k] * a[k];
      break;
    case RB200_OP_INVERT:
#pragma unroll
      for (int k = 0; k < V; ++k) r[k] = (I.imm() == 1) ? (a[k] == 0 ? 1 : 0) : ~a[k];
      break;
    case RB200_OP_LNOT:
#pragma unroll
      for (int k = 0; k < V; ++k) r[k] = a[k] == 0 ? 1 : 0;
      break;
    case RB200_OP_ISFINITE:
#pragma unroll
      for (int k = 0; k < V; ++k) r[k] = 1;
      break;
    case RB200_OP_ISINF:
    case RB200_OP_ISNAN:
    case RB200_OP_ISNEGINF:
    case RB200_OP_ISPOSINF:
#pragma unroll
      for (int k = 0; k < V; ++k) r[k] = 0;
      break;
    case RB200_OP_WHERE: {
      long long c[V];
      cx.template fetch<long long>(I.c_kind(), I.c_idx(), c);
#pragma unroll
      for (int k = 0; k < V; ++k) r[k] = (a[k] != 0) ? b[k] : c[k];
    } break;
    case RB200_OP_MULADD:
    case RB200_OP_MULSUB:
    case RB200_OP_MULRSUB: {
      long long c[V];
      cx.template fetch<long long>(I.c_kind(), I.c_idx(), c);
#pragma unroll
      for (int k = 0; k < V; ++k) {
        const long long p = b[k] * c[k];
        r[k] = op == RB200_OP_MULADD ? a[k] + p : op == RB200_OP_MULSUB ? a[k] - p : p - a[k];
      }
    } break;
    default: return;
  }
  cx.template finish<long long>(I, r);
}

template <class T> __device__ __forceinline__ T through_storage(T x, int dt) {
  switch (dt) {
    case RB200_F64: return (T)(double)x;
    case RB200_F32: return (T)(float)x;
    case RB200_I64: return (T)(long long)x;
    case RB200_I32: return (T)(int)x;
    case RB200_BOOL: return (T)(x != T(0) ? 1 : 0);
    case RB200_U8: return (T)(unsigned char)(long long)x;
    case RB200_I8: return (T)(signed char)(long long)x;
    case RB200_I16: return (T)(short)(long long)x;
    case RB200_U16: return (T)(unsigned short)(long long)x;
    case RB200_U32: return (T)(unsigned int)(long long)x;
    default: return x;
  }
}

template <class S, int V, class C> __device__ __forceinline__ void exec_cvt_from(C& cx, const UInsn& I) {
  S a[V];
  cx.template fetch<S>(I.a_kind(), I.a_idx(), a);
  const int through = (int)(I.imm() >> 8);
  if (through != 0) {
#pragma unroll
    for (int k = 0; k < V; ++k) a[k] = through_storage<S>(a[k], through - 1);
  }
  switch (I.ctype()) {
    case RB200_T_F64: {
      double r[V];
#pragma unroll
      for (int k = 0; k < V; ++k) r[k] = (double)a[k];
      cx.template finish<double>(I, r);
    } break;
    case RB200_T_F32: {
      float r[V];
#pragma unroll
      for (int k = 0; k < V; ++k) r[k] = (float)a[k];
      cx.template finish<float>(I, r);
    } break;
    default: {
      long long r[V];
#pragma unroll
      for (int k = 0; k < V; ++k) r[k] = (long long)a[k];
      cx.template finish<long long>(I, r);
    }
  }
}

template <class T, int SK, int V, class C> __device__ __forceinline__ void fetch_s(C& cx, int i, T (&out)[V]) {
  if constexpr (SK == S_ACC) {
#pragma unroll
    for (int k = 0; k < V; ++k) out[k] = CT<T>::get(cx.acc[k]);
  } else if constexpr (SK == S_REG) {
    lds_vec64<T, V>(cx.reg_base(i), out);
  } else if constexpr (SK == S_SCAL) {
    const T s = CT<T>::get(cx.P.scalars[i]);
#pragma unroll
    for (int k = 0; k < V; ++k) out[k] = s;
  } else if constexpr (SK == S_PFV) {
    const unsigned slot_s = cx.pf_s + (unsigned)(i * V * kThreads * 8);
    if constexpr (sizeof(T) == 8) lds_vec64<T, V>(slot_s + cx.tid * 8u, out);
    else lds_vec32<T, V>(slot_s + cx.tid * 4u, out);
  } else if constexpr (SK == S_PFV32) {
    const unsigned slot_s = cx.pf_s + (unsigned)(i * V * kThreads * 8);
    if constexpr (std::is_same<T, double>::value) lds_vec32_as_f64<V>(slot_s + cx.tid * 4u, out);
  } else if constexpr (SK == S_VIEW) {
    const KView& vw = cx.P.views[i];
    long long off[V];
    cx.offsets(vw, off);
    load_direct<T, T, V>(vw.base, off, cx.valid, out);
  } else {
    const KView& vw = cx.P.views[i];
    long long off[V];
    cx.offsets(vw, off);
    if constexpr (std::is_same<T, double>::value) load_direct<double, float, V>(vw.base, off, cx.valid, out);
  }
}

template <int OP, class T, int AK, int BK, int V, class C> __device__ __forceinline__ void h_bin(C& cx, const UInsn& I) {
  T a[V], b[V], r[V];
  fetch_s<T, AK, V>(cx, I.a_idx(), a);
  fetch_s<T, BK, V>(cx, I.b_idx(), b);
#pragma unroll
  for (int k = 0; k < V; ++k) {
    if constexpr (sizeof(T) == 8 && !std::is_integral<T>::value) {
      r[k] = OP == RB200_OP_ADD ? __dadd_rn(a[k], b[k]) : OP == RB200_OP_SUB ? __dsub_rn(a[k], b[k]) : __dmul_rn(a[k], b[k]);
    } else if constexpr (sizeof(T) == 4) {
      r[k] = OP == RB200_OP_ADD ? __fadd_rn(a[k], b[k]) : OP == RB200_OP_SUB ? __fsub_rn(a[k], b[k]) : __fmul_rn(a[k], b[k]);
    } else {
      r[k] = OP == RB200_OP_ADD ? a[k] + b[k] : OP == RB200_OP_SUB ? a[k] - b[k] : a[k] * b[k];
    }
  }
  cx.template finish<T>(I, r);
}

template <int OP, class T, int AK, int V, class C> __device__ __forceinline__ void h_un(C& cx, const UInsn& I) {
  T a[V], r[V];
  fetch_s<T, AK, V>(cx, I.a_idx(), a);
  if constexpr (OP == RB200_OP_SIN || OP == RB200_OP_COS || OP == RB200_OP_SINCOS) {
    if constexpr (!std::is_integral<T>::value) {
      T sn[V], cs[V];
      sincos_v<V>(a, sn, cs);
      const bool want_cos = (OP == RB200_OP_COS) || (OP == RB200_OP_SINCOS && I.imm());
#pragma unroll
      for (int k = 0; k < V; ++k) r[k] = want_cos ? cs[k] : sn[k];
      if constexpr (OP == RB200_OP_SINCOS) {
        u64 park[V];
        T parkv[V];
#pragma unroll
        for (int k = 0; k < V; ++k) {
          parkv[k] = want_cos ? sn[k] : cs[k];
          park[k] = CT<T>::bits(parkv[k]);
        }
        sts_vec64<V>(cx.reg_base(I.st2()), park);
        if (I.c_kind() == RB200_K_VIEW) cx.template store_res<T>(I.c_idx(), RB200_NOSTORE, parkv, park);
      }
    }
    cx.template finish<T>(I, r);
    return;
  }
#pragma unroll
  for (int k = 0; k < V; ++k) {
    if constexpr (OP == RB200_OP_MOV) r[k] = a[k];
    else if constexpr (OP == RB200_OP_NEG) r[k] = -a[k];
    else if constexpr (OP == RB200_OP_ABS) {
      if constexpr (std::is_integral<T>::value) r[k] = a[k] < 0 ? -a[k] : a[k];
      else r[k] = fabs(a[k]);
    } else if constexpr (OP == RB200_OP_SQUARE || OP == RB200_OP_POWI) {
      if constexpr (std::is_integral<T>::value) r[k] = a[k] * a[k];
      else if constexpr (sizeof(T) == 8) r[k] = __dmul_rn(a[k], a[k]);
      else r[k] = __fmul_rn(a[k], a[k]);
    } else if constexpr (OP == RB200_OP_SQRT) r[k] = sqrt(a[k]);
    else if constexpr (OP == RB200_OP_SIN) r[k] = sin(a[k]);
    else if constexpr (OP == RB200_OP_COS) r[k] = cos(a[k]);
    else if constexpr (OP == RB200_OP_SINCOS) {
      T sn, cs;
      sincos(a[k], &sn, &cs);
      r[k] = I.imm() ? cs : sn;
      sts64(cx.reg_addr(I.st2(), k), CT<T>::bits(I.imm() ? sn : cs));
    }
  }
  cx.template finish<T>(I, r);
}

template <class TS, class TD, int AK, int V, class C> __device__ __forceinline__ void h_cvt(C& cx, const UInsn& I) {
  TS a[V];
  TD r[V];
  fetch_s<TS, AK, V>(cx, I.a_idx(), a);
#pragma unroll
  for (int k = 0; k < V; ++k) r[k] = (TD)a[k];
  cx.template finish<TD>(I, r);
}

template <class T, int AK, int V, bool AX, int NS, class C>
__device__ __forceinline__ void h_red(C& cx, const UInsn& I, u64 (&racc)[NS][AX ? V : 1]) {
  T a[V];
  fetch_s<T, AK, V>(cx, I.a_idx(), a);
  const int slot = I.b_idx();
  const int rop = (int)I.imm();
  if constexpr (!AX) {
    const T ident = CT<T>::get(red_identity_bits(rop, std::is_integral<T>::value ? RB200_T_I64 : RB200_T_F64));
    if (cx.valid != ((1u << V) - 1u)) {
#pragma unroll
      for (int k = 0; k < V; ++k)
        if (!((cx.valid >> k) & 1u)) a[k] = ident;
    }
    if (rop == RB200_RED_ADD) {
#pragma unroll
      for (int w = V / 2; w >= 1; w >>= 1)
#pragma unroll
        for (int k = 0; k < w; ++k) a[k] = a[k] + a[k + w];
    } else {
#pragma unroll
      for (int w = V / 2; w >= 1; w >>= 1)
#pragma unroll
        for (int k = 0; k < w; ++k) a[k] = red_combine<T>(rop, a[k], a[k + w]);
    }
    if (slot == 0) {
      racc[0][0] = CT<T>::bits(red_combine<T>(rop, CT<T>::get(racc[0][0]), a[0]));
    } else {
      const unsigned addr = cx.racc_s + (unsigned)(slot - 1) * (unsigned)(kThreads * 8);
      sts64(addr, CT<T>::bits(red_combine<T>(rop, CT<T>::get(lds64(addr)), a[0])));
    }
  } else {
#pragma unroll
    for (int s = 0; s < NS; ++s)
      if (s == slot) {
#pragma unroll
        for (int k = 0; k < V; ++k)
          if ((cx.valid >> k) & 1u) {
            u64& t = racc[s][k];
            t = CT<T>::bits(red_combine<T>(rop, CT<T>::get(t), a[k]));
          }
      }
  }
}

template <class R, int V, class C> __device__ __forceinline__ void finish_bits(C& cx, const UInsn& I, const u64 (&b)[V]) {
  R r[V];
#pragma unroll
  for (int k = 0; k < V; ++k) r[k] = CT<R>::get(b[k]);
  cx.template finish<R>(I, r);
}
template <int V, class C> __device__ __forceinline__ void exec_philox(C& cx, const UInsn& I) {
  long long a[V];
  cx.template fetch<long long>(I.a_kind(), I.a_idx(), a);
  const u64 key = cx.P.scalars[I.b_idx()];
  const u64 n = I.c_kind() == RB200_K_SCAL ? cx.P.scalars[I.c_idx()] : 1ull;
  const unsigned form = I.imm();
  u64 b[V];
#pragma unroll
  for (int k = 0; k < V; ++k) b[k] = philox_element_bits(a[k], key, n, form);
  switch (I.ctype()) {
    case RB200_T_F64: finish_bits<double, V>(cx, I, b); break;
    case RB200_T_F32: finish_bits<float, V>(cx, I, b); break;
    default: finish_bits<long long, V>(cx, I, b);
  }
}

template <int V, bool AX, int NS, class C> __device__ __forceinline__ void generic_body(C& cx, const UInsn& I, u64 (&racc)[NS][AX ? V : 1]) {
  if (I.op() == RB200_OP_PHILOX) {
    exec_philox<V>(cx, I);
    return;
  }
  if (I.op() == RB200_OP_CVT) {
    switch (I.imm() & 0xff) {
      case RB200_T_F64: exec_cvt_from<double, V>(cx, I); break;
      case RB200_T_F32: exec_cvt_from<float, V>(cx, I); break;
      default: exec_cvt_from<long long, V>(cx, I);
    }
    return;
  }
  if (I.op() == RB200_OP_RED) {
    const int slot = I.b_idx();
    const int rop = (int)I.imm();
    if (I.ctype() == RB200_T_F64) {
      double a[V];
      cx.template fetch<double>(I.a_kind(), I.a_idx(), a);
      if constexpr (AX) {
#pragma unroll
        for (int s = 0; s < NS; ++s)
          if (s == slot) {
#pragma unroll
            for (int k = 0; k < V; ++k)
              if ((cx.valid >> k) & 1u) {
                u64& t = racc[s][AX ? k : 0];
                t = CT<double>::bits(red_combine<double>(rop, CT<double>::get(t), a[k]));
              }
          }
      } else {
        const unsigned addr = cx.racc_s + (unsigned)(slot - 1) * (unsigned)(kThreads * 8);
        u64 t = slot == 0 ? racc[0][0] : lds64(addr);
#pragma unroll
        for (int k = 0; k < V; ++k)
          if ((cx.valid >> k) & 1u) t = CT<double>::bits(red_combine<double>(rop, CT<double>::get(t), a[k]));
        if (slot == 0) racc[0][0] = t;
        else sts64(addr, t);
      }
    } else {
      long long a[V];
      cx.template fetch<long long>(I.a_kind(), I.a_idx(), a);
      if constexpr (AX) {
#pragma unroll
        for (int s = 0; s < NS; ++s)
          if (s == slot) {
#pragma unroll
            for (int k = 0; k < V; ++k)
              if ((cx.valid >> k) & 1u) {
                u64& t = racc[s][AX ? k : 0];
                t = (u64)red_combine<long long>(rop, (long long)t, a[k]);
              }
          }
      } else {
        const unsigned addr = cx.racc_s + (unsigned)(slot - 1) * (unsigned)(kThreads * 8);
        u64 t = slot == 0 ? racc[0][0] : lds64(addr);
#pragma unroll
        for (int k = 0; k < V; ++k)
          if ((cx.valid >> k) & 1u) t = (u64)red_combine<long long>(rop, (long long)t, a[k]);
        if (slot == 0) racc[0][0] = t;
        else sts64(addr, t);
      }
    }
    return;
  }
  switch (I.ctype()) {
    case RB200_T_F64: exec_float<double, V>(cx, I); break;
    case RB200_T_F32: exec_float<float, V>(cx, I); break;
    default: exec_int<V>(cx, I);
  }
}

#ifndef RB200_NO_FAST_HANDLERS
template <int V, bool AX, int NS, class C> __device__ __noinline__ void generic_step(C cx, int pc, u64* acc_out, u64* racc_io) {
  u64 racc[NS][AX ? V : 1];
#pragma unroll
  for (int s = 0; s < NS; ++s)
#pragma unroll
    for (int k = 0; k < (AX ? V : 1); ++k) racc[s][k] = racc_io[s * (AX ? V : 1) + k];
  const UInsn I(&cx.P.insns[pc]);
  generic_body<V, AX, NS>(cx, I, racc);
#pragma unroll
  for (int k = 0; k < V; ++k) acc_out[k] = cx.acc[k];
#pragma unroll
  for (int s = 0; s < NS; ++s)
#pragma unroll
    for (int k = 0; k < (AX ? V : 1); ++k) racc_io[s * (AX ? V : 1) + k] = racc[s][k];
}
#endif

template <int V, bool AX, int NS, class C> __device__ __forceinline__ void run_program(C& cx, u64 (&racc)[NS][AX ? V : 1]) {
  const KParams& P = cx.P;
  const int n = P.n_insns;
  const unsigned valid_tile = cx.valid;
#pragma unroll 1
  for (int pc = 0; pc < n; ++pc) {
    const UInsn I(&P.insns[pc]);
    {
      unsigned v = valid_tile;
      if constexpr (C::kND == 1) asm volatile("" : "+r"(v));
      cx.valid = v;
    }
#ifndef RB200_NO_FAST_HANDLERS
    const int h = P.handler[pc];
    if (h != H_GENERIC) {
#if RB200_HANDLER_SET == 2
#include "rb200_handlers_set2.inc"
#else
#include "rb200_handlers_set1.inc"
#endif
      continue;
    }
    {
      u64 acc_tmp[V], racc_tmp[NS * (AX ? V : 1)];
#pragma unroll
      for (int s = 0; s < NS; ++s)
#pragma unroll
        for (int k = 0; k < (AX ? V : 1); ++k) racc_tmp[s * (AX ? V : 1) + k] = racc[s][k];
      generic_step<V, AX, NS, C>(cx, pc, acc_tmp, racc_tmp);
#pragma unroll
      for (int k = 0; k < V; ++k) cx.acc[k] = acc_tmp[k];
#pragma unroll
      for (int s = 0; s < NS; ++s)
#pragma unroll
        for (int k = 0; k < (AX ? V : 1); ++k) racc[s][k] = racc_tmp[s * (AX ? V : 1) + k];
    }
#else
    generic_body<V, AX, NS>(cx, I, racc);
#endif
  }
}

template <int ND> __device__ __forceinline__ void decode_index(const KParams& P, long long e, int d0, long long (&idx)[ND]) {
#pragma unroll
  for (int d = ND - 1; d >= 0; --d) {
    if (d >= P.ndim || d < d0) {
      if (d < d0) continue;
      idx[d] = 0;
      continue;
    }
    if (d == d0) {
      idx[d] = e;
    } else {
      const long long sd = P.shape[d];
      long long q;
      if (((e | sd) >> 31) == 0) q = (long long)((unsigned)e / (unsigned)sd);
      else q = e / sd;
      idx[d] = e - q * sd;
      e = q;
    }
  }
}

}
```

### ramba_b200/csrc/rb200_launch.h

```cpp
#pragma once
#include "rb200_vm.cuh"

namespace rb200 {
constexpr int kV = 4;
constexpr int kV1 = 8;
cudaError_t launch_vm_elementwise_nd1(const KParams& P, unsigned blocks, size_t smem, cudaStream_t stream);
cudaError_t launch_vm_elementwise_nd2(const KParams& P, unsigned blocks, size_t smem, cudaStream_t stream);
cudaError_t launch_vm_elementwise_nd3(const KParams& P, unsigned blocks, size_t smem, cudaStream_t stream);
cudaError_t launch_vm_elementwise_nd5(const KParams& P, unsigned blocks, size_t smem, cudaStream_t stream);
cudaError_t launch_vm_elementwise_ax1d(const KParams& P, unsigned blocks, size_t smem, cudaStream_t stream);
cudaError_t launch_vm_axis_reduce(const KParams& P, unsigned blocks, size_t smem, cudaStream_t stream);
long long scan_scratch_bytes(long long n_outer, long long len, long long n_inner);
cudaError_t launch_scan(const void* src, void* dst, int dtype, long long n_outer, long long len, long long n_inner, int op, const void* carry, void* totals,
                        void* scratch, int sms, cudaStream_t stream, bool* supported);
}
```

Before: 2548.

## Add lean 1-D interpreter kernel variant with pruned handler switch

Adds a specialized 1-D elementwise kernel instantiation (LEAN) used when every instruction maps to a reduced handler set (f64/f32, common ops, contiguous own-dtype stores, no reductions, no masks). The lean kernel compiles a smaller dispatch switch, drops the generic fallback, skips reduction setup and epilogue, stores directly with plain global stores, and uses less shared memory. The intent is to cut register pressure and code size in the interpreter loop so occupancy and instruction throughput improve. It adds a new kernel binary and an eligibility check that must stay consistent with the handler tables.

Result: faster. 2642 (median of 6 runs) (+3.7%).

```diff
diff --git a/ramba_b200/csrc/gen_handlers.py b/ramba_b200/csrc/gen_handlers.py
--- a/ramba_b200/csrc/gen_handlers.py
+++ b/ramba_b200/csrc/gen_handlers.py
@@ -5,6 +5,11 @@
 UN = ["RB200_OP_MOV", "RB200_OP_NEG", "RB200_OP_ABS", "RB200_OP_SQUARE", "RB200_OP_SQRT", "RB200_OP_SIN", "RB200_OP_COS",
       "RB200_OP_SINCOS", "RB200_OP_POWI"]
 FLOAT_ONLY = {"RB200_OP_SQRT", "RB200_OP_SIN", "RB200_OP_COS", "RB200_OP_SINCOS", "RB200_OP_POWI"}
+LEAN_OPS = {"RB200_OP_MOV", "RB200_OP_NEG", "RB200_OP_ABS", "RB200_OP_SQUARE", "RB200_OP_SIN", "RB200_OP_COS", "RB200_OP_SINCOS",
+            "RB200_OP_POWI", "RB200_OP_ADD", "RB200_OP_SUB", "RB200_OP_MUL"}
+LEAN_T = {"double", "float"}
+LEAN_AK = {"S_ACC", "S_REG", "S_PFV"}
+LEAN_BK = {"S_ACC", "S_REG", "S_SCAL", "S_PFV"}
 
 SETS = {
     1: dict(AK=["S_ACC", "S_REG", "S_PFV", "S_PFV32"], BK=["S_ACC", "S_REG", "S_SCAL", "S_PFV", "S_PFV32"]),
@@ -18,11 +23,30 @@
     return str(x)
 
 
+def write_switch(path, cases):
+    groups = {}
+    for n, stmt in cases:
+        groups.setdefault(n >> 4, []).append((n & 15, stmt))
+    lines = ["// GENERATED by gen_handlers.py — do not edit", "switch (h >> 4) {"]
+    for gi in sorted(groups):
+        lines.append(f"  case {gi}:")
+        lines.append("    switch (h & 15) {")
+        for lo, stmt in groups[gi]:
+            lines.append(f"      case {lo}: {stmt}")
+        lines.append("      default: break;")
+        lines.append("    }")
+        lines.append("    break;")
+    lines.append("  default: break;")
+    lines.append("}")
+    open(path, "w").write("\n".join(lines) + "\n")
+
+
 tab = ["// GENERATED by gen_handlers.py — do not edit", "#pragma once", "namespace rb200 {"]
 for sid, kinds in SETS.items():
     AK, BK = kinds["AK"], kinds["BK"]
     wide32 = {AK[3], BK[4]}
     cases = []
+    lean = []
     hid = 0
     hbin = [[[[0] * len(BK) for _ in AK] for _ in T] for _ in BIN]
     hun = [[[0] * len(AK) for _ in T] for _ in UN]
@@ -40,6 +64,8 @@
                             hid += 1
                             hbin[oi][ti][ai][bi] = hid
                             cases.append((hid, f"h_bin<{op}, {t}, {ak}, {bk}, V>(cx, I); break;"))
+                            if op in LEAN_OPS and t in LEAN_T and ak in LEAN_AK and bk in LEAN_BK:
+                                lean.append(len(cases) - 1)
                 continue
             for oi, op in enumerate(UN):
                 if not group(op):
@@ -52,6 +78,8 @@
                     hid += 1
                     hun[oi][ti][ai] = hid
                     cases.append((hid, f"h_un<{op}, {t}, {ak}, V>(cx, I); break;"))
+                    if op in LEAN_OPS and t in LEAN_T and ak in LEAN_AK:
+                        lean.append(len(cases) - 1)
     for ti, t in enumerate(["double", "long long"]):
         for ai, ak in enumerate(AK):
             if ak in wide32 and t != "double":
@@ -67,21 +95,7 @@
                 hid += 1
                 hcvt[si][di][ai] = hid
                 cases.append((hid, f"h_cvt<{ts}, {td}, {ak}, V>(cx, I); break;"))
-    groups = {}
-    for n, stmt in cases:
-        groups.setdefault(n >> 4, []).append((n & 15, stmt))
-    lines = ["// GENERATED by gen_handlers.py — do not edit", "switch (h >> 4) {"]
-    for gi in sorted(groups):
-        lines.append(f"  case {gi}:")
-        lines.append("    switch (h & 15) {")
-        for lo, stmt in groups[gi]:
-            lines.append(f"      case {lo}: {stmt}")
-        lines.append("      default: break;")
-        lines.append("    }")
-        lines.append("    break;")
-    lines.append("  default: break;")
-    lines.append("}")
-    open(f"rb200_handlers_set{sid}.inc", "w").write("\n".join(lines) + "\n")
+    write_switch(f"rb200_handlers_set{sid}.inc", cases)
     tab += [f"// ---- set {sid}: a kinds {AK}, b kinds {BK}",
             f"constexpr int kNumHandlers{sid} = {hid};",
             f"static const short kHandlerBin{sid}[{len(BIN)}][{len(T)}][{len(AK)}][{len(BK)}] = {carr(hbin)};",
@@ -89,5 +103,16 @@
             f"static const short kHandlerRed{sid}[2][{len(AK)}] = {carr(hred)};",
             f"static const short kHandlerCvt{sid}[{len(T)}][{len(T)}][{len(AK)}] = {carr(hcvt)};"]
     print("set", sid, hid, "handlers")
+    if sid == 1:
+        lean_of = [0] * (hid + 1)
+        lean_cases = []
+        for j, ci in enumerate(lean):
+            lean_of[cases[ci][0]] = j + 1
+            lean_cases.append((j + 1, cases[ci][1]))
+        write_switch("rb200_handlers_lean.inc", lean_cases)
+        tab += [f"// ---- lean set: set-1 handler id -> lean handler id (0: not in the lean set)",
+                f"constexpr int kNumHandlersLean = {len(lean)};",
+                f"static const unsigned char kLeanOf1[{hid + 1}] = {carr(lean_of)};"]
+        print("lean", len(lean), "handlers")
 tab += ["}  // namespace rb200", ""]
 open("rb200_handler_tables.h", "w").write("\n".join(tab))
diff --git a/ramba_b200/csrc/rb200_api.cu b/ramba_b200/csrc/rb200_api.cu
--- a/ramba_b200/csrc/rb200_api.cu
+++ b/ramba_b200/csrc/rb200_api.cu
@@ -140,13 +140,13 @@
 }
 
 struct KillSwitches {
-  bool no_tile, no_stream, no_mapred, no_terms, no_tma, no_row_mode, no_rng;
+  bool no_tile, no_stream, no_mapred, no_terms, no_tma, no_row_mode, no_rng, no_lean;
 };
 static const KillSwitches& kill_switches() {
   static const KillSwitches k = {getenv("RB200_NO_TILE_KERNEL") != nullptr,   getenv("RB200_NO_STREAM_KERNEL") != nullptr,
                                  getenv("RB200_NO_MAPRED_KERNEL") != nullptr, getenv("RB200_NO_TERMS_KERNEL") != nullptr,
                                  getenv("RB200_NO_TMA") != nullptr,           getenv("RB200_NO_ROW_MODE") != nullptr,
-                                 getenv("RB200_NO_RNG") != nullptr};
+                                 getenv("RB200_NO_RNG") != nullptr,           getenv("RB200_NO_LEAN_INTERP") != nullptr};
   return k;
 }
 
@@ -234,6 +234,7 @@
   StreamPlan stream;
   RngPlan rng;
   KParams k;
+  bool lean;
   long long blocks;
   size_t smem;
   int n_split, n_written;
@@ -336,9 +337,25 @@
   return true;
 }
 
+static bool lean_eligible(const KParams& P, const rb200_fused_op* op) {
+  if (P.ndim != 1 || op->n_reds != 0 || (P.n_pf > 0 && !P.bulk)) return false;
+  for (int i = 0; i < P.n_insns; ++i) {
+    const rb200_insn& I = P.insns[i];
+    const int h = P.handler[i];
+    if (h == H_GENERIC || kLeanOf1[h] == 0) return false;
+    if (I.st_view != RB200_NOSTORE && I.mask_reg != RB200_NOSTORE) return false;
+    const int own = I.ctype == RB200_T_F64 ? RB200_F64 : RB200_F32;
+    const int stored[2] = {I.st_view, (I.op == RB200_OP_SINCOS && I.c_kind == RB200_K_VIEW) ? (int)I.c_idx : RB200_NOSTORE};
+    for (const int v : stored)
+      if (v != RB200_NOSTORE && (P.views[v].stride[0] != 1 || P.views[v].dtype != own)) return false;
+  }
+  return true;
+}
+
 static void make_plan(const rb200_fused_op* op, int sms, Plan& pl) {
   const KillSwitches& ks = kill_switches();
   pl.form = FORM_NONE;
+  pl.lean = false;
   pl.n_split = pl.n_written = 0;
   if (!ks.no_rng && plan_rng(op, sms, pl.rng)) {
     pl.form = FORM_RNG;
@@ -478,8 +495,12 @@
     }
     ocls_bytes = (size_t)P.n_ocls * V * kThreads * 8;
   }
-  const size_t smem = reg_bytes + pf_bytes + ocls_bytes;
   assign_handlers(P, op, op->ndim == 1 ? 1 : 2);
+  if (!ks.no_lean && lean_eligible(P, op)) {
+    pl.lean = true;
+    for (int i = 0; i < P.n_insns; ++i) P.handler[i] = kLeanOf1[P.handler[i]];
+  }
+  const size_t smem = (pl.lean ? reg_bytes - (size_t)V * kThreads * 8 : reg_bytes) + pf_bytes + ocls_bytes;
   if (op->n_reds > 0) {
     P.red_counter = (unsigned int*)op->red_scratch;
     P.red_partials = (u64*)((char*)op->red_scratch + 256);
@@ -522,8 +543,8 @@
     case FORM_AXIS_AS_1D: return "vm_elementwise_kernel (axis-as-1-D) launch";
     case FORM_AXIS_REDUCE: return "vm_axis_reduce_kernel launch";
     default:
-      snprintf(buf, sizeof(buf), "vm_elementwise_kernel launch (ndim=%d blocks=%lld smem=%zu n_regs=%d n_pf=%d n_insns=%d)", P.ndim, pl.blocks, pl.smem,
-               P.n_regs, P.n_pf, P.n_insns);
+      snprintf(buf, sizeof(buf), "vm_elementwise_kernel%s launch (ndim=%d blocks=%lld smem=%zu n_regs=%d n_pf=%d n_insns=%d)", pl.lean ? " (lean)" : "", P.ndim,
+               pl.blocks, pl.smem, P.n_regs, P.n_pf, P.n_insns);
   }
   return buf;
 }
@@ -541,7 +562,7 @@
     case FORM_AXIS_REDUCE: e = launch_vm_axis_reduce(P, blocks, pl.smem, stream); break;
     case FORM_ELEMENTWISE:
       switch (P.ndim) {
-        case 1: e = launch_vm_elementwise_nd1(P, blocks, pl.smem, stream); break;
+        case 1: e = pl.lean ? launch_vm_elementwise_lean(P, blocks, pl.smem, stream) : launch_vm_elementwise_nd1(P, blocks, pl.smem, stream); break;
         case 2: e = launch_vm_elementwise_nd2(P, blocks, pl.smem, stream); break;
         case 3: e = launch_vm_elementwise_nd3(P, blocks, pl.smem, stream); break;
         default: e = launch_vm_elementwise_nd5(P, blocks, pl.smem, stream); break;
@@ -569,8 +590,8 @@
   const char* form = pl.form == FORM_ELEMENTWISE ? "elementwise" : pl.form == FORM_AXIS_AS_1D ? "axis_as_1d" : "axis_reduce";
   const char* tiling = pl.form != FORM_ELEMENTWISE || op->ndim == 1 ? "" : pl.k.row_chunks > 0 ? " tiling=row" : " tiling=flat";
   char buf[200];
-  snprintf(buf, sizeof(buf), "kernel=general_interpreter form=%s ndim=%d insns=%d views=%d%s ctas=%lld smem=%zu", form, op->ndim, op->n_insns, op->n_views,
-           tiling, pl.blocks, pl.smem);
+  snprintf(buf, sizeof(buf), "kernel=general_interpreter form=%s ndim=%d insns=%d views=%d%s ctas=%lld smem=%zu%s", form, op->ndim, op->n_insns,
+           op->n_views, tiling, pl.blocks, pl.smem, pl.lean ? " variant=lean" : "");
   return buf;
 }
 
diff --git a/ramba_b200/csrc/rb200_elementwise.cuh b/ramba_b200/csrc/rb200_elementwise.cuh
--- a/ramba_b200/csrc/rb200_elementwise.cuh
+++ b/ramba_b200/csrc/rb200_elementwise.cuh
@@ -4,22 +4,23 @@
 
 namespace rb200 {
 
-template <int V, int ND, bool AX1D = false>
+template <int V, int ND, bool AX1D = false, bool LEAN = false>
 #ifndef RB200_MIN_BLOCKS
 #define RB200_MIN_BLOCKS 2
 #endif
 __global__ void __launch_bounds__(kThreads, (ND == 1 && V <= 4) ? 3 : RB200_MIN_BLOCKS) vm_elementwise_kernel(const __grid_constant__ KParams P) {
+  static_assert(!LEAN || (ND == 1 && !AX1D), "the lean kernel is the plain 1-D one");
   extern __shared__ __align__(128) unsigned char smem[];
   __shared__ __align__(8) u64 mbar_store[4];
   constexpr int TILE = kThreads * V;
   constexpr unsigned SLOT = (unsigned)(TILE * 8);
-  Ctx<V, ND> cx(P);
+  Ctx<V, ND, LEAN> cx(P);
   const unsigned smem_s = (unsigned)__cvta_generic_to_shared(smem);
   cx.tid = threadIdx.x;
   const int n_pf = (ND == 1) ? P.n_pf : 0;
   const unsigned pf_base = smem_s;
   const unsigned pf_stage_bytes = (unsigned)n_pf * SLOT;
-  const bool bulk = (ND == 1) && n_pf > 0 && P.bulk;
+  const bool bulk = (ND == 1) && n_pf > 0 && (LEAN || P.bulk);
   constexpr unsigned S = 2u;
   cx.regfile_s = smem_s + (n_pf > 0 ? S : 0u) * pf_stage_bytes + threadIdx.x * 8u;
   cx.ocls_s = cx.regfile_s + (unsigned)((P.n_regs + 1) * V * kThreads * 8);
@@ -36,10 +37,12 @@
   constexpr int NS = 1;
   __shared__ u64 racc_extra[RB200_MAX_REDS - 1][kThreads];
   u64 racc[NS][AX1D ? V : 1];
-#pragma unroll
-  for (int k = 0; k < (AX1D ? V : 1); ++k) racc[0][k] = red_identity_bits(0 < P.n_reds ? P.reds[0].op : 0, 0 < P.n_reds ? P.reds[0].ctype : 0);
-  cx.racc_s = (unsigned)__cvta_generic_to_shared(&racc_extra[0][threadIdx.x]);
-  for (int s = 1; s < P.n_reds; ++s) racc_extra[s - 1][threadIdx.x] = red_identity_bits(P.reds[s].op, P.reds[s].ctype);
+  if constexpr (!LEAN) {
+#pragma unroll
+    for (int k = 0; k < (AX1D ? V : 1); ++k) racc[0][k] = red_identity_bits(0 < P.n_reds ? P.reds[0].op : 0, 0 < P.n_reds ? P.reds[0].ctype : 0);
+    cx.racc_s = (unsigned)__cvta_generic_to_shared(&racc_extra[0][threadIdx.x]);
+    for (int s = 1; s < P.n_reds; ++s) racc_extra[s - 1][threadIdx.x] = red_identity_bits(P.reds[s].op, P.reds[s].ctype);
+  }
   if constexpr (AX1D) {
     cx.pe0 = (long long)(blockIdx.x % (unsigned)P.n_split_chunks) * TILE + threadIdx.x;
     cx.e0 = cx.pe0;
@@ -210,8 +213,9 @@
     }
     cx.valid = valid;
     cx.fill_offset_classes();
-    run_program<V, AX1D, NS>(cx, racc);
-  }
+    run_program<V, AX1D, NS, LEAN>(cx, racc);
+  }
+  if constexpr (LEAN) return;
   if (n_pf > 0 && !bulk) cp_async_wait<0>();
 
   if constexpr (AX1D) {
@@ -282,12 +286,13 @@
   }
 }
 
-template <int V, int ND, bool AX1D = false> cudaError_t launch_vm_elementwise_nd(const KParams& P, unsigned blocks, size_t smem, cudaStream_t stream) {
+template <int V, int ND, bool AX1D = false, bool LEAN = false>
+cudaError_t launch_vm_elementwise_nd(const KParams& P, unsigned blocks, size_t smem, cudaStream_t stream) {
   if (smem + 2048 > 48 * 1024) {
-    cudaError_t e = cudaFuncSetAttribute(vm_elementwise_kernel<V, ND, AX1D>, cudaFuncAttributeMaxDynamicSharedMemorySize, (int)smem);
+    cudaError_t e = cudaFuncSetAttribute(vm_elementwise_kernel<V, ND, AX1D, LEAN>, cudaFuncAttributeMaxDynamicSharedMemorySize, (int)smem);
     if (e != cudaSuccess) return e;
   }
-  vm_elementwise_kernel<V, ND, AX1D><<<blocks, kThreads, smem, stream>>>(P);
+  vm_elementwise_kernel<V, ND, AX1D, LEAN><<<blocks, kThreads, smem, stream>>>(P);
   return cudaGetLastError();
 }
 
diff --git a/ramba_b200/csrc/rb200_elementwise_lean.cu b/ramba_b200/csrc/rb200_elementwise_lean.cu
--- /dev/null
+++ b/ramba_b200/csrc/rb200_elementwise_lean.cu
@@ -0,0 +1,6 @@
+#include "rb200_elementwise.cuh"
+namespace rb200 {
+cudaError_t launch_vm_elementwise_lean(const KParams& P, unsigned blocks, size_t smem, cudaStream_t stream) {
+  return launch_vm_elementwise_nd<kV1, 1, false, true>(P, blocks, smem, stream);
+}
+}
diff --git a/ramba_b200/csrc/rb200_handler_tables.h b/ramba_b200/csrc/rb200_handler_tables.h
--- a/ramba_b200/csrc/rb200_handler_tables.h
+++ b/ramba_b200/csrc/rb200_handler_tables.h
@@ -5,6 +5,8 @@
 static const short kHandlerUn1[9][3][4] = {{{1, 2, 3, 4}, {97, 98, 99, 0}, {160, 161, 162, 0}}, {{5, 6, 7, 8}, {100, 101, 102, 0}, {163, 164, 165, 0}}, {{9, 10, 11, 12}, {103, 104, 105, 0}, {166, 167, 168, 0}}, {{13, 14, 15, 16}, {106, 107, 108, 0}, {169, 170, 171, 0}}, {{17, 18, 19, 20}, {109, 110, 111, 0}, {0, 0, 0, 0}}, {{85, 86, 87, 88}, {151, 152, 153, 0}, {0, 0, 0, 0}}, {{89, 90, 91, 92}, {154, 155, 156, 0}, {0, 0, 0, 0}}, {{93, 94, 95, 96}, {157, 158, 159, 0}, {0, 0, 0, 0}}, {{21, 22, 23, 24}, {112, 113, 114, 0}, {0, 0, 0, 0}}};
 static const short kHandlerRed1[2][4] = {{208, 209, 210, 211}, {212, 213, 214, 0}};
 static const short kHandlerCvt1[3][3][4] = {{{0, 0, 0, 0}, {215, 216, 217, 0}, {218, 219, 220, 0}}, {{221, 222, 223, 0}, {0, 0, 0, 0}, {224, 225, 226, 0}}, {{227, 228, 229, 0}, {230, 231, 232, 0}, {0, 0, 0, 0}}};
+constexpr int kNumHandlersLean = 120;
+static const unsigned char kLeanOf1[233] = {0, 1, 2, 3, 0, 4, 5, 6, 0, 7, 8, 9, 0, 10, 11, 12, 0, 0, 0, 0, 0, 13, 14, 15, 0, 16, 17, 18, 19, 0, 20, 21, 22, 23, 0, 24, 25, 26, 27, 0, 0, 0, 0, 0, 0, 28, 29, 30, 31, 0, 32, 33, 34, 35, 0, 36, 37, 38, 39, 0, 0, 0, 0, 0, 0, 40, 41, 42, 43, 0, 44, 45, 46, 47, 0, 48, 49, 50, 51, 0, 0, 0, 0, 0, 0, 52, 53, 54, 0, 55, 56, 57, 0, 58, 59, 60, 0, 61, 62, 63, 64, 65, 66, 67, 68, 69, 70, 71, 72, 0, 0, 0, 73, 74, 75, 76, 77, 78, 79, 80, 81, 82, 83, 84, 85, 86, 87, 88, 89, 90, 91, 92, 93, 94, 95, 96, 97, 98, 99, 100, 101, 102, 103, 104, 105, 106, 107, 108, 109, 110, 111, 112, 113, 114, 115, 116, 117, 118, 119, 120, 0, 0, 0, 0, 0, 0, 0, 0, 0, 0, 0, 0, 0, 0, 0, 0, 0, 0, 0, 0, 0, 0, 0, 0, 0, 0, 0, 0, 0, 0, 0, 0, 0, 0, 0, 0, 0, 0, 0, 0, 0, 0, 0, 0, 0, 0, 0, 0, 0, 0, 0, 0, 0, 0, 0, 0, 0, 0, 0, 0, 0, 0, 0, 0, 0, 0, 0, 0, 0, 0, 0, 0, 0};
 constexpr int kNumHandlers2 = 232;
 static const short kHandlerBin2[3][3][4][5] = {{{{25, 26, 27, 28, 29}, {30, 31, 32, 33, 34}, {35, 36, 37, 38, 39}, {40, 41, 42, 43, 44}}, {{115, 116, 117, 118, 0}, {119, 120, 121, 122, 0}, {123, 124, 125, 126, 0}, {0, 0, 0, 0, 0}}, {{172, 173, 174, 175, 0}, {176, 177, 178, 179, 0}, {180, 181, 182, 183, 0}, {0, 0, 0, 0, 0}}}, {{{45, 46, 47, 48, 49}, {50, 51, 52, 53, 54}, {55, 56, 57, 58, 59}, {60, 61, 62, 63, 64}}, {{127, 128, 129, 130, 0}, {131, 132, 133, 134, 0}, {135, 136, 137, 138, 0}, {0, 0, 0, 0, 0}}, {{184, 185, 186, 187, 0}, {188, 189, 190, 191, 0}, {192, 193, 194, 195, 0}, {0, 0, 0, 0, 0}}}, {{{65, 66, 67, 68, 69}, {70, 71, 72, 73, 74}, {75, 76, 77, 78, 79}, {80, 81, 82, 83, 84}}, {{139, 140, 141, 142, 0}, {143, 144, 145, 146, 0}, {147, 148, 149, 150, 0}, {0, 0, 0, 0, 0}}, {{196, 197, 198, 199, 0}, {200, 201, 202, 203, 0}, {204, 205, 206, 207, 0}, {0, 0, 0, 0, 0}}}};
 static const short kHandlerUn2[9][3][4] = {{{1, 2, 3, 4}, {97, 98, 99, 0}, {160, 161, 162, 0}}, {{5, 6, 7, 8}, {100, 101, 102, 0}, {163, 164, 165, 0}}, {{9, 10, 11, 12}, {103, 104, 105, 0}, {166, 167, 168, 0}}, {{13, 14, 15, 16}, {106, 107, 108, 0}, {169, 170, 171, 0}}, {{17, 18, 19, 20}, {109, 110, 111, 0}, {0, 0, 0, 0}}, {{85, 86, 87, 88}, {151, 152, 153, 0}, {0, 0, 0, 0}}, {{89, 90, 91, 92}, {154, 155, 156, 0}, {0, 0, 0, 0}}, {{93, 94, 95, 96}, {157, 158, 159, 0}, {0, 0, 0, 0}}, {{21, 22, 23, 24}, {112, 113, 114, 0}, {0, 0, 0, 0}}};
diff --git a/ramba_b200/csrc/rb200_handlers_lean.inc b/ramba_b200/csrc/rb200_handlers_lean.inc
--- /dev/null
+++ b/ramba_b200/csrc/rb200_handlers_lean.inc
@@ -0,0 +1,163 @@
+switch (h >> 4) {
+  case 0:
+    switch (h & 15) {
+      case 1: h_un<RB200_OP_MOV, double, S_ACC, V>(cx, I); break;
+      case 2: h_un<RB200_OP_MOV, double, S_REG, V>(cx, I); break;
+      case 3: h_un<RB200_OP_MOV, double, S_PFV, V>(cx, I); break;
+      case 4: h_un<RB200_OP_NEG, double, S_ACC, V>(cx, I); break;
+      case 5: h_un<RB200_OP_NEG, double, S_REG, V>(cx, I); break;
+      case 6: h_un<RB200_OP_NEG, double, S_PFV, V>(cx, I); break;
+      case 7: h_un<RB200_OP_ABS, double, S_ACC, V>(cx, I); break;
+      case 8: h_un<RB200_OP_ABS, double, S_REG, V>(cx, I); break;
+      case 9: h_un<RB200_OP_ABS, double, S_PFV, V>(cx, I); break;
+      case 10: h_un<RB200_OP_SQUARE, double, S_ACC, V>(cx, I); break;
+      case 11: h_un<RB200_OP_SQUARE, double, S_REG, V>(cx, I); break;
+      case 12: h_un<RB200_OP_SQUARE, double, S_PFV, V>(cx, I); break;
+      case 13: h_un<RB200_OP_POWI, double, S_ACC, V>(cx, I); break;
+      case 14: h_un<RB200_OP_POWI, double, S_REG, V>(cx, I); break;
+      case 15: h_un<RB200_OP_POWI, double, S_PFV, V>(cx, I); break;
+      default: break;
+    }
+    break;
+  case 1:
+    switch (h & 15) {
+      case 0: h_bin<RB200_OP_ADD, double, S_ACC, S_ACC, V>(cx, I); break;
+      case 1: h_bin<RB200_OP_ADD, double, S_ACC, S_REG, V>(cx, I); break;
+      case 2: h_bin<RB200_OP_ADD, double, S_ACC, S_SCAL, V>(cx, I); break;
+      case 3: h_bin<RB200_OP_ADD, double, S_ACC, S_PFV, V>(cx, I); break;
+      case 4: h_bin<RB200_OP_ADD, double, S_REG, S_ACC, V>(cx, I); break;
+      case 5: h_bin<RB200_OP_ADD, double, S_REG, S_REG, V>(cx, I); break;
+      case 6: h_bin<RB200_OP_ADD, double, S_REG, S_SCAL, V>(cx, I); break;
+      case 7: h_bin<RB200_OP_ADD, double, S_REG, S_PFV, V>(cx, I); break;
+      case 8: h_bin<RB200_OP_ADD, double, S_PFV, S_ACC, V>(cx, I); break;
+      case 9: h_bin<RB200_OP_ADD, double, S_PFV, S_REG, V>(cx, I); break;
+      case 10: h_bin<RB200_OP_ADD, double, S_PFV, S_SCAL, V>(cx, I); break;
+      case 11: h_bin<RB200_OP_ADD, double, S_PFV, S_PFV, V>(cx, I); break;
+      case 12: h_bin<RB200_OP_SUB, double, S_ACC, S_ACC, V>(cx, I); break;
+      case 13: h_bin<RB200_OP_SUB, double, S_ACC, S_REG, V>(cx, I); break;
+      case 14: h_bin<RB200_OP_SUB, double, S_ACC, S_SCAL, V>(cx, I); break;
+      case 15: h_bin<RB200_OP_SUB, double, S_ACC, S_PFV, V>(cx, I); break;
+      default: break;
+    }
+    break;
+  case 2:
+    switch (h & 15) {
+      case 0: h_bin<RB200_OP_SUB, double, S_REG, S_ACC, V>(cx, I); break;
+      case 1: h_bin<RB200_OP_SUB, double, S_REG, S_REG, V>(cx, I); break;
+      case 2: h_bin<RB200_OP_SUB, double, S_REG, S_SCAL, V>(cx, I); break;
+      case 3: h_bin<RB200_OP_SUB, double, S_REG, S_PFV, V>(cx, I); break;
+      case 4: h_bin<RB200_OP_SUB, double, S_PFV, S_ACC, V>(cx, I); break;
+      case 5: h_bin<RB200_OP_SUB, double, S_PFV, S_REG, V>(cx, I); break;
+      case 6: h_bin<RB200_OP_SUB, double, S_PFV, S_SCAL, V>(cx, I); break;
+      case 7: h_bin<RB200_OP_SUB, double, S_PFV, S_PFV, V>(cx, I); break;
+      case 8: h_bin<RB200_OP_MUL, double, S_ACC, S_ACC, V>(cx, I); break;
+      case 9: h_bin<RB200_OP_MUL, double, S_ACC, S_REG, V>(cx, I); break;
+      case 10: h_bin<RB200_OP_MUL, double, S_ACC, S_SCAL, V>(cx, I); break;
+      case 11: h_bin<RB200_OP_MUL, double, S_ACC, S_PFV, V>(cx, I); break;
+      case 12: h_bin<RB200_OP_MUL, double, S_REG, S_ACC, V>(cx, I); break;
+      case 13: h_bin<RB200_OP_MUL, double, S_REG, S_REG, V>(cx, I); break;
+      case 14: h_bin<RB200_OP_MUL, double, S_REG, S_SCAL, V>(cx, I); break;
+      case 15: h_bin<RB200_OP_MUL, double, S_REG, S_PFV, V>(cx, I); break;
+      default: break;
+    }
+    break;
+  case 3:
+    switch (h & 15) {
+      case 0: h_bin<RB200_OP_MUL, double, S_PFV, S_ACC, V>(cx, I); break;
+      case 1: h_bin<RB200_OP_MUL, double, S_PFV, S_REG, V>(cx, I); break;
+      case 2: h_bin<RB200_OP_MUL, double, S_PFV, S_SCAL, V>(cx, I); break;
+      case 3: h_bin<RB200_OP_MUL, double, S_PFV, S_PFV, V>(cx, I); break;
+      case 4: h_un<RB200_OP_SIN, double, S_ACC, V>(cx, I); break;
+      case 5: h_un<RB200_OP_SIN, double, S_REG, V>(cx, I); break;
+      case 6: h_un<RB200_OP_SIN, double, S_PFV, V>(cx, I); break;
+      case 7: h_un<RB200_OP_COS, double, S_ACC, V>(cx, I); break;
+      case 8: h_un<RB200_OP_COS, double, S_REG, V>(cx, I); break;
+      case 9: h_un<RB200_OP_COS, double, S_PFV, V>(cx, I); break;
+      case 10: h_un<RB200_OP_SINCOS, double, S_ACC, V>(cx, I); break;
+      case 11: h_un<RB200_OP_SINCOS, double, S_REG, V>(cx, I); break;
+      case 12: h_un<RB200_OP_SINCOS, double, S_PFV, V>(cx, I); break;
+      case 13: h_un<RB200_OP_MOV, float, S_ACC, V>(cx, I); break;
+      case 14: h_un<RB200_OP_MOV, float, S_REG, V>(cx, I); break;
+      case 15: h_un<RB200_OP_MOV, float, S_PFV, V>(cx, I); break;
+      default: break;
+    }
+    break;
+  case 4:
+    switch (h & 15) {
+      case 0: h_un<RB200_OP_NEG, float, S_ACC, V>(cx, I); break;
+      case 1: h_un<RB200_OP_NEG, float, S_REG, V>(cx, I); break;
+      case 2: h_un<RB200_OP_NEG, float, S_PFV, V>(cx, I); break;
+      case 3: h_un<RB200_OP_ABS, float, S_ACC, V>(cx, I); break;
+      case 4: h_un<RB200_OP_ABS, float, S_REG, V>(cx, I); break;
+      case 5: h_un<RB200_OP_ABS, float, S_PFV, V>(cx, I); break;
+      case 6: h_un<RB200_OP_SQUARE, float, S_ACC, V>(cx, I); break;
+      case 7: h_un<RB200_OP_SQUARE, float, S_REG, V>(cx, I); break;
+      case 8: h_un<RB200_OP_SQUARE, float, S_PFV, V>(cx, I); break;
+      case 9: h_un<RB200_OP_POWI, float, S_ACC, V>(cx, I); break;
+      case 10: h_un<RB200_OP_POWI, float, S_REG, V>(cx, I); break;
+      case 11: h_un<RB200_OP_POWI, float, S_PFV, V>(cx, I); break;
+      case 12: h_bin<RB200_OP_ADD, float, S_ACC, S_ACC, V>(cx, I); break;
+      case 13: h_bin<RB200_OP_ADD, float, S_ACC, S_REG, V>(cx, I); break;
+      case 14: h_bin<RB200_OP_ADD, float, S_ACC, S_SCAL, V>(cx, I); break;
+      case 15: h_bin<RB200_OP_ADD, float, S_ACC, S_PFV, V>(cx, I); break;
+      default: break;
+    }
+    break;
+  case 5:
+    switch (h & 15) {
+      case 0: h_bin<RB200_OP_ADD, float, S_REG, S_ACC, V>(cx, I); break;
+      case 1: h_bin<RB200_OP_ADD, float, S_REG, S_REG, V>(cx, I); break;
+      case 2: h_bin<RB200_OP_ADD, float, S_REG, S_SCAL, V>(cx, I); break;
+      case 3: h_bin<RB200_OP_ADD, float, S_REG, S_PFV, V>(cx, I); break;
+      case 4: h_bin<RB200_OP_ADD, float, S_PFV, S_ACC, V>(cx, I); break;
+      case 5: h_bin<RB200_OP_ADD, float, S_PFV, S_REG, V>(cx, I); break;
+      case 6: h_bin<RB200_OP_ADD, float, S_PFV, S_SCAL, V>(cx, I); break;
+      case 7: h_bin<RB200_OP_ADD, float, S_PFV, S_PFV, V>(cx, I); break;
+      case 8: h_bin<RB200_OP_SUB, float, S_ACC, S_ACC, V>(cx, I); break;
+      case 9: h_bin<RB200_OP_SUB, float, S_ACC, S_REG, V>(cx, I); break;
+      case 10: h_bin<RB200_OP_SUB, float, S_ACC, S_SCAL, V>(cx, I); break;
+      case 11: h_bin<RB200_OP_SUB, float, S_ACC, S_PFV, V>(cx, I); break;
+      case 12: h_bin<RB200_OP_SUB, float, S_REG, S_ACC, V>(cx, I); break;
+      case 13: h_bin<RB200_OP_SUB, float, S_REG, S_REG, V>(cx, I); break;
+      case 14: h_bin<RB200_OP_SUB, float, S_REG, S_SCAL, V>(cx, I); break;
+      case 15: h_bin<RB200_OP_SUB, float, S_REG, S_PFV, V>(cx, I); break;
+      default: break;
+    }
+    break;
+  case 6:
+    switch (h & 15) {
+      case 0: h_bin<RB200_OP_SUB, float, S_PFV, S_ACC, V>(cx, I); break;
+      case 1: h_bin<RB200_OP_SUB, float, S_PFV, S_REG, V>(cx, I); break;
+      case 2: h_bin<RB200_OP_SUB, float, S_PFV, S_SCAL, V>(cx, I); break;
+      case 3: h_bin<RB200_OP_SUB, float, S_PFV, S_PFV, V>(cx, I); break;
+      case 4: h_bin<RB200_OP_MUL, float, S_ACC, S_ACC, V>(cx, I); break;
+      case 5: h_bin<RB200_OP_MUL, float, S_ACC, S_REG, V>(cx, I); break;
+      case 6: h_bin<RB200_OP_MUL, float, S_ACC, S_SCAL, V>(cx, I); break;
+      case 7: h_bin<RB200_OP_MUL, float, S_ACC, S_PFV, V>(cx, I); break;
+      case 8: h_bin<RB200_OP_MUL, float, S_REG, S_ACC, V>(cx, I); break;
+      case 9: h_bin<RB200_OP_MUL, float, S_REG, S_REG, V>(cx, I); break;
+      case 10: h_bin<RB200_OP_MUL, float, S_REG, S_SCAL, V>(cx, I); break;
+      case 11: h_bin<RB200_OP_MUL, float, S_REG, S_PFV, V>(cx, I); break;
+      case 12: h_bin<RB200_OP_MUL, float, S_PFV, S_ACC, V>(cx, I); break;
+      case 13: h_bin<RB200_OP_MUL, float, S_PFV, S_REG, V>(cx, I); break;
+      case 14: h_bin<RB200_OP_MUL, float, S_PFV, S_SCAL, V>(cx, I); break;
+      case 15: h_bin<RB200_OP_MUL, float, S_PFV, S_PFV, V>(cx, I); break;
+      default: break;
+    }
+    break;
+  case 7:
+    switch (h & 15) {
+      case 0: h_un<RB200_OP_SIN, float, S_ACC, V>(cx, I); break;
+      case 1: h_un<RB200_OP_SIN, float, S_REG, V>(cx, I); break;
+      case 2: h_un<RB200_OP_SIN, float, S_PFV, V>(cx, I); break;
+      case 3: h_un<RB200_OP_COS, float, S_ACC, V>(cx, I); break;
+      case 4: h_un<RB200_OP_COS, float, S_REG, V>(cx, I); break;
+      case 5: h_un<RB200_OP_COS, float, S_PFV, V>(cx, I); break;
+      case 6: h_un<RB200_OP_SINCOS, float, S_ACC, V>(cx, I); break;
+      case 7: h_un<RB200_OP_SINCOS, float, S_REG, V>(cx, I); break;
+      case 8: h_un<RB200_OP_SINCOS, float, S_PFV, V>(cx, I); break;
+      default: break;
+    }
+    break;
+  default: break;
+}
diff --git a/ramba_b200/csrc/rb200_interp.cuh b/ramba_b200/csrc/rb200_interp.cuh
--- a/ramba_b200/csrc/rb200_interp.cuh
+++ b/ramba_b200/csrc/rb200_interp.cuh
@@ -105,7 +105,7 @@
   if (mask & 8u) store_one<R>(base, dtype, o3, CT<R>::get(lds64(vals_addr + (unsigned)(3 * kThreads * 8))));
 }
 
-template <int V, int ND> struct Ctx {
+template <int V, int ND, bool LEAN = false> struct Ctx {
   static constexpr int kND = ND;
   const KParams& P;
   unsigned regfile_s;
@@ -259,7 +259,17 @@
   }
 
   template <class R> __device__ __forceinline__ void store_res(int vi, int mreg, const R (&r)[V], const u64 (&b)[V]) {
-    if constexpr (ND == 1 && (V == 4 || V == 8)) {
+    if constexpr (LEAN) {
+      R* p = reinterpret_cast<R*>(P.views[vi].base) + e0;
+      if (valid == ((1u << V) - 1u)) {
+#pragma unroll
+        for (int k = 0; k < V; ++k) stg<R>(p + k * kThreads, r[k]);
+      } else {
+#pragma unroll
+        for (int k = 0; k < V; ++k)
+          if ((valid >> k) & 1u) stg<R>(p + k * kThreads, r[k]);
+      }
+    } else if constexpr (ND == 1 && (V == 4 || V == 8)) {
       const KView& vw = P.views[vi];
       constexpr int own1 = std::is_same<R, double>::value ? RB200_F64 : std::is_same<R, float>::value ? RB200_F32 : RB200_I64;
       const long long st = vw.stride[0];
@@ -984,7 +994,7 @@
 }
 #endif
 
-template <int V, bool AX, int NS, class C> __device__ __forceinline__ void run_program(C& cx, u64 (&racc)[NS][AX ? V : 1]) {
+template <int V, bool AX, int NS, bool LEAN = false, class C> __device__ __forceinline__ void run_program(C& cx, u64 (&racc)[NS][AX ? V : 1]) {
   const KParams& P = cx.P;
   const int n = P.n_insns;
   const unsigned valid_tile = cx.valid;
@@ -998,27 +1008,31 @@
     }
 #ifndef RB200_NO_FAST_HANDLERS
     const int h = P.handler[pc];
-    if (h != H_GENERIC) {
+    if constexpr (LEAN) {
+#include "rb200_handlers_lean.inc"
+    } else {
+      if (h != H_GENERIC) {
 #if RB200_HANDLER_SET == 2
 #include "rb200_handlers_set2.inc"
 #else
 #include "rb200_handlers_set1.inc"
 #endif
-      continue;
-    }
-    {
-      u64 acc_tmp[V], racc_tmp[NS * (AX ? V : 1)];
-#pragma unroll
-      for (int s = 0; s < NS; ++s)
-#pragma unroll
-        for (int k = 0; k < (AX ? V : 1); ++k) racc_tmp[s * (AX ? V : 1) + k] = racc[s][k];
-      generic_step<V, AX, NS, C>(cx, pc, acc_tmp, racc_tmp);
-#pragma unroll
-      for (int k = 0; k < V; ++k) cx.acc[k] = acc_tmp[k];
-#pragma unroll
-      for (int s = 0; s < NS; ++s)
-#pragma unroll
-        for (int k = 0; k < (AX ? V : 1); ++k) racc[s][k] = racc_tmp[s * (AX ? V : 1) + k];
+        continue;
+      }
+      {
+        u64 acc_tmp[V], racc_tmp[NS * (AX ? V : 1)];
+#pragma unroll
+        for (int s = 0; s < NS; ++s)
+#pragma unroll
+          for (int k = 0; k < (AX ? V : 1); ++k) racc_tmp[s * (AX ? V : 1) + k] = racc[s][k];
+        generic_step<V, AX, NS, C>(cx, pc, acc_tmp, racc_tmp);
+#pragma unroll
+        for (int k = 0; k < V; ++k) cx.acc[k] = acc_tmp[k];
+#pragma unroll
+        for (int s = 0; s < NS; ++s)
+#pragma unroll
+          for (int k = 0; k < (AX ? V : 1); ++k) racc[s][k] = racc_tmp[s * (AX ? V : 1) + k];
+      }
     }
 #else
     generic_body<V, AX, NS>(cx, I, racc);
diff --git a/ramba_b200/csrc/rb200_launch.h b/ramba_b200/csrc/rb200_launch.h
--- a/ramba_b200/csrc/rb200_launch.h
+++ b/ramba_b200/csrc/rb200_launch.h
@@ -8,6 +8,7 @@
 cudaError_t launch_vm_elementwise_nd2(const KParams& P, unsigned blocks, size_t smem, cudaStream_t stream);
 cudaError_t launch_vm_elementwise_nd3(const KParams& P, unsigned blocks, size_t smem, cudaStream_t stream);
 cudaError_t launch_vm_elementwise_nd5(const KParams& P, unsigned blocks, size_t smem, cudaStream_t stream);
+cudaError_t launch_vm_elementwise_lean(const KParams& P, unsigned blocks, size_t smem, cudaStream_t stream);
 cudaError_t launch_vm_elementwise_ax1d(const KParams& P, unsigned blocks, size_t smem, cudaStream_t stream);
 cudaError_t launch_vm_axis_reduce(const KParams& P, unsigned blocks, size_t smem, cudaStream_t stream);
 long long scan_scratch_bytes(long long n_outer, long long len, long long n_inner);
```
